# beecave-homelab/VibeVoice-ROCm

Measured on AMD Instinct MI355X. Metric: audio-sec/s, higher is better.
Workload: dtype bf16; 1 GPU; cfg2: VibeVoice-1.5B shapes, 1 speaker(s) x 203-frame voice prompt, 330-token prompt, 225 frames (30.0 s audio), CFG=2.0, 20 DPM-Solver++ steps, whole generate() incl. voice encode + prefill; global_batch=1, parallelism=replicas x1 (one dialogue per GPU), hipgraph=True

## Files before the change

### include/vv_hip.h

```cpp
#ifndef VV_HIP_H
#define VV_HIP_H

#include <stddef.h>
#include <stdint.h>

#ifdef __cplusplus
extern "C" {
#endif

typedef void* vv_stream_t;

enum { VV_F32 = 0, VV_BF16 = 1, VV_FP8 = 2  };
enum { VV_NF4 = 3 };
enum { VV_WQ_NF4 = 0x100 };
enum { VV_MXFP4 = 4 };
enum { VV_WQ_MXFP4 = 0x200 };
enum { VV_MXFP4_FRAG = 5 };
enum { VV_WQ_FRAG4 = 0x400 };
enum { VV_MXFP6 = 6 };
enum { VV_WQ_MXFP6 = 0x800 };
enum { VV_MXFP6_FRAG = 8 };
enum { VV_WQ_FRAG6 = 0x1000 };
enum { VV_OK = 0, VV_E_ARG = -1, VV_E_HIP = -2, VV_E_UNSUPPORTED = -3 };
enum { VV_PRO_NONE = 0, VV_PRO_RMSNORM = 1, VV_PRO_SILU = 2 };
// ... 122 lines not shown
                       const vv_sampler* sampler, const float* q, vv_stream_t stream);
int vv_llm_tail_batch_sample(const vv_llm* m, const float* h, int64_t ldh, int B, float* out, int64_t ldo, const void* w_valid, int nv, const int* ids,
                             float* logits_out, int* token_out, const int* forced_token, int* lens, int tok_start, int tok_diffusion,
                             int* frame_counter, const int* active, const vv_sampler* sampler, const float* q, vv_stream_t stream);
int vv_sample_ids(const float* logits, int n, const int* ids, const vv_sampler* sampler, const float* q, int* token_out, const int* forced_token,
                  vv_stream_t stream);

int vv_token_draws(float* q, int64_t ldq, int B, int nv, const uint64_t* seeds, const int* pos, int64_t ld_pos, int pos_bias, vv_stream_t stream);
int vv_llm_tail_sample_rows(const vv_llm* m, const float* h, int64_t ldh, int R, float* out, int64_t ldo, const void* w_valid, int nv, const int* ids,
                            float* logits_out, int* token_out, const int* forced_token, int* lens, int tok_start, int tok_diffusion, int* frame_counter,
                            const vv_sampler* samplers, const uint64_t* seeds, vv_stream_t stream);
int vv_llm_tail_batch_sample_rows(const vv_llm* m, const float* h, int64_t ldh, int B, float* out, int64_t ldo, const void* w_valid, int nv, const int* ids,
                                  float* logits_out, int* token_out, const int* forced_token, int* lens, int tok_start, int tok_diffusion,
                                  int* frame_counter, const int* active, const vv_sampler* samplers, const uint64_t* seeds, vv_stream_t stream);

typedef struct vv_head_layer {
  const float* norm_w;
  const void* wgate;
  const void* wup;
  const void* wdown;
  const void* adaln;
  vv_w8 q_gate, q_up, q_down;
  const void* f_gate; const void* f_up; const void* f_down;
} vv_head_layer;

typedef struct vv_head {
  int wdt, D, ffn, layers, latent, cond_dim;
  float eps;
  int flags;
  const void* noisy_proj;
  const void* cond_proj;
  const void* final_adaln;
  const void* final_linear;
  const vv_head_layer* layer;
  const float* fused_g;
} vv_head;

typedef struct vv_dpm_coef { float alpha_s, sigma_s, cx, cd, rinv; int order; float cn;  } vv_dpm_coef;

int vv_add_rows_silu(const float* a, int64_t lda, const float* b, int64_t ldb, float* out, int rows, int rows_b, int n, vv_stream_t stream);
int vv_add_rows_silu_bf16(const float* a, int64_t lda, const float* b, int64_t ldb, void* out, int rows, int rows_b, int n, vv_stream_t stream);
int vv_dpm_proj(const float* v, int64_t ldv, float cfg_scale, const vv_dpm_coef* coef, const float* x_in, const float* m_in,
                float* x_out, float* m_out, const void* w, int wdt, int latent, int D, float* h, int64_t ldh, int rows,
                const float* step_noise , vv_stream_t stream);

size_t vv_head_ws_bytes(const vv_head* h, int n_steps);
int vv_head_sample(const vv_head* h, const float* cond2, int64_t ld_cond, const float* noise, const float* temb,
                   const vv_dpm_coef* coef, int n_steps, float cfg_scale, float* latent_out, void* ws,
                   const float* sde_noise ,
                   vv_stream_t stream);
size_t vv_head_ws_bytes_batch(const vv_head* h, int n_steps, int B);
int vv_head_sample_batch(const vv_head* h, const float* cond, int64_t ld_cond, const float* noise, int64_t ld_noise, const float* temb,
                         const vv_dpm_coef* coef, int n_steps, float cfg_scale, float* latent_out, int64_t ld_latent, int B, void* ws,
                         vv_stream_t stream);
size_t vv_head_ws_bytes_batch_sde(const vv_head* h, int n_steps, int B);
int vv_head_sample_batch_sde(const vv_head* h, const float* cond, int64_t ld_cond, const float* noise, int64_t ld_noise, const float* temb,
                             const vv_dpm_coef* coef, int n_steps, float cfg_scale, float* latent_out, int64_t ld_latent, int B, void* ws,
                             const float* sde_noise, int64_t ld_sde, vv_stream_t stream);
int vv_head_sample_batch_cfg(const vv_head* h, const float* cond, int64_t ld_cond, const float* noise, int64_t ld_noise, const float* temb,
                             const vv_dpm_coef* coef, int n_steps, const float* cfg_rows , float* latent_out, int64_t ld_latent,
                             int B, void* ws, const float* sde_noise , int64_t ld_sde, vv_stream_t stream);
int vv_head_sample_route(const vv_head* h, const float* cond, int64_t ld_cond, const float* temb, const vv_dpm_coef* coef, int n_steps, int B,
                         int sde, const float* cfg_rows, const void* ws, char* name, int cap);
int vv_head_ws_layout(const vv_head* h, int n_steps, int B, int sde, int64_t* off, int cap);
int vv_noise_normal(float* noise, int64_t ld_noise, float* sde_noise, int64_t ld_sde, int B, int n, int n_steps, const uint64_t* seeds,
                    const int* frames, vv_stream_t stream);
int vv_head_forward(const vv_head* h, const float* x, const float* temb_rows, const float* cond, int R, float* v,
                    void* ws, vv_stream_t stream);

typedef struct vv_block {
  const float* gamma; const float* ffn_gamma; const float* norm_w; const float* ffn_norm_w;
  const float* dw_w;
  const float* dw_b;
  const void* w1; const float* b1;
  const void* w2; const float* b2;
  float* hist;
  vv_w8 q_w1, q_w2;
  const float* dw_last;
  float* hs;
} vv_block;

int vv_block1d(const struct vv_block* b, int wdt, const float* x, float* out, int T, int C, float eps, vv_stream_t stream);
int vv_block1d_route(const struct vv_block* b, int wdt, const float* x, const float* out, int T, int C, char* name, int cap);

size_t vv_block_mid_ws_bytes(int T, int C);
int vv_block_mid(const struct vv_block* b, int wdt, const float* x, float* out, void* ws, int T, int C, float eps, vv_stream_t stream);
int vv_block_mid_route(const struct vv_block* b, int wdt, const float* x, const float* out, const void* ws, int T, int C, char* name, int cap);

typedef struct vv_conv {
  const void* w;
  const float* b;
  int cin, cout, kk, stride, transposed;
  float* state;
} vv_conv;

#define VV_MAX_STAGES 8
typedef struct vv_convnet {
  int wdt, n_stages;
  float eps;
  vv_conv sample[VV_MAX_STAGES];
  int n_blocks[VV_MAX_STAGES];
  const vv_block* blocks[VV_MAX_STAGES];
  vv_conv head;
} vv_convnet;

size_t vv_convnet_ws_bytes(const vv_convnet* net, int64_t t_in, int decoder);
int vv_decoder_forward(const vv_convnet* net, const float* latent, int T, float pre_scale, float pre_bias, float* wav,
                       void* ws, vv_stream_t stream);
int vv_encoder_forward(const vv_convnet* net, const float* wav, int64_t T, float* feat, void* ws, vv_stream_t stream);
int vv_convnet_reset(const vv_convnet* net, vv_stream_t stream);

typedef struct vv_connector { int wdt, din, hidden; const void* fc1; const float* b1; const float* norm_w; const void* fc2; const float* b2; } vv_connector;
int vv_connector_forward(const vv_connector* c, const float* x, int R, float* out, int accumulate, float* ws, vv_stream_t stream);
int vv_connector_pair(const vv_connector* ac, const vv_connector* sem, const float* latent, const float* semfeat, float* out, int64_t ldo,
                      int rows_out, float* ws, vv_stream_t stream);

size_t vv_conv_rows_ws_bytes(const vv_convnet* net, int B, int decoder);
int vv_decoder_front_rows(const vv_convnet* const* nets, int B, const int* active, const float* latent, int64_t ld_latent,
                          float pre_scale, float pre_bias, float* mid, int64_t ld_mid, void* ws, vv_stream_t stream);
int vv_decoder_forward_from(const vv_convnet* net, const float* mid, float* wav, void* ws, vv_stream_t stream);
int vv_encoder_forward_until(const vv_convnet* net, const float* wav, int64_t T, float* mid, void* ws, vv_stream_t stream);
int vv_encoder_back_rows(const vv_convnet* const* nets, int B, const int* active, const float* mid, int64_t ld_mid,
                         float* feat, int64_t ld_feat, void* ws, vv_stream_t stream);
int vv_connector_pair_rows(const vv_connector* ac, const vv_connector* sem, const float* latent, int64_t ld_latent,
                           const float* semfeat, int64_t ld_feat, const int* active, float* out, int64_t ld_out,
                           int rows_out, int B, float* ws, vv_stream_t stream);

int vv_graph_begin(vv_stream_t stream);
int vv_graph_end(vv_stream_t stream, void** graph_exec_out);
int vv_graph_launch(void* graph_exec, vv_stream_t stream);
int vv_graph_destroy(void* graph_exec);

typedef struct vv_prof_entry { int m, n, k, dual, wdt, count; double total_ms; } vv_prof_entry;
int vv_prof_begin(int max_records);
int vv_prof_end(vv_prof_entry* out, int max_out, int* n_out);

typedef struct vv_nf4_src {
  const uint8_t* packed;
  const void* absmax;
  const float* quant_map;
  const float* nested_absmax;
  const float* nested_map;
  float nested_offset;
  int nested_blocksize;
  int n, k, blocksize;
} vv_nf4_src;
int vv_nf4_import(const vv_nf4_src* src, void* w, int64_t ldw, int row0, int rows_total, void* cq, float* cs, vv_stream_t stream);

#define VV_CONV_HOT_GEMV 0
#define VV_CONV_HOT_ROW 1
typedef struct vv_conv_hot_shape { const char* name; int kind, m, n, k, bias, gate, res; } vv_conv_hot_shape;
int vv_conv_hot_shapes(vv_conv_hot_shape* out, int cap);

size_t vv_sizeof(const char* struct_name);

#ifdef __cplusplus
}
#endif
#endif
```

### vibevoice_rocm_amd/_lib.py

```python
from __future__ import annotations

import ctypes as C
import os

_HERE = os.path.dirname(os.path.abspath(__file__))
LIB_PATH = os.path.join(_HERE, "libvv_hip.so")

VV_F32, VV_BF16, VV_FP8, VV_NF4, VV_MXFP4, VV_MXFP4_FRAG, VV_MXFP6 = 0, 1, 2, 3, 4, 5, 6
VV_MXFP6_FRAG = 8
VV_WQ_NF4 = 0x100
VV_WQ_MXFP4 = 0x200
VV_WQ_MXFP6 = 0x800
VV_WQ_FRAG4 = 0x400
VV_WQ_FRAG6 = 0x1000
PRO_NONE, PRO_RMSNORM, PRO_SILU = 0, 1, 2
ACT_NONE, ACT_GELU, ACT_SWIGLU = 0, 1, 2
LIN_X_BF16, LIN_OUT_BF16, LIN_W_REUSED, LIN_W_FRAG, LIN_PACKED, LIN_W_MXGEMM = 1, 2, 4, 8, 16, 32
LIN_W_MX6GEMM = 64
VV_MAX_STAGES = 8
KVQ_DERIVE_SCALES = 1

vp = C.c_void_p
i64 = C.c_int64

# ... 17 lines not shown

def kv_fp8_scale(absmax: float) -> float:
    import math
    a = abs(float(absmax))
    if a == 0.0:
        return 1.0
    m, e = math.frexp(a)
    return math.ldexp(1.0, e - 8 if m <= 0.875 else e - 7)


class LlmLayer(C.Structure):
    _fields_ = [("ln1", vp), ("ln2", vp), ("wqkv", vp), ("bqkv", vp), ("wo", vp), ("wgate", vp), ("wup", vp), ("wdown", vp),
                ("q_qkv", W8), ("q_o", W8), ("q_gate", W8), ("q_up", W8), ("q_down", W8),
                ("f_qkv", vp), ("f_o", vp), ("f_gate", vp), ("f_up", vp), ("f_down", vp)]


class Llm(C.Structure):
    _fields_ = [("wdt", C.c_int), ("hidden", C.c_int), ("inter", C.c_int), ("layers", C.c_int), ("heads", C.c_int),
                ("kv_heads", C.c_int), ("head_dim", C.c_int), ("rms_eps", C.c_float), ("inv_freq", vp),
                ("final_norm", vp), ("layer", C.POINTER(LlmLayer))]


class HeadLayer(C.Structure):
    _fields_ = [("norm_w", vp), ("wgate", vp), ("wup", vp), ("wdown", vp), ("adaln", vp), ("q_gate", W8), ("q_up", W8), ("q_down", W8),
                ("f_gate", vp), ("f_up", vp), ("f_down", vp)]


class Head(C.Structure):
    _fields_ = [("wdt", C.c_int), ("D", C.c_int), ("ffn", C.c_int), ("layers", C.c_int), ("latent", C.c_int),
                ("cond_dim", C.c_int), ("eps", C.c_float), ("flags", C.c_int), ("noisy_proj", vp), ("cond_proj", vp), ("final_adaln", vp),
                ("final_linear", vp), ("layer", C.POINTER(HeadLayer)), ("fused_g", vp)]


class DpmCoef(C.Structure):
    _fields_ = [("alpha_s", C.c_float), ("sigma_s", C.c_float), ("cx", C.c_float), ("cd", C.c_float),
                ("rinv", C.c_float), ("order", C.c_int), ("cn", C.c_float)]


class Block(C.Structure):
    _fields_ = [("gamma", vp), ("ffn_gamma", vp), ("norm_w", vp), ("ffn_norm_w", vp), ("dw_w", vp), ("dw_b", vp),
                ("w1", vp), ("b1", vp), ("w2", vp), ("b2", vp), ("hist", vp), ("q_w1", W8), ("q_w2", W8), ("dw_last", vp), ("hs", vp)]


class Conv(C.Structure):
    _fields_ = [("w", vp), ("b", vp), ("cin", C.c_int), ("cout", C.c_int), ("kk", C.c_int), ("stride", C.c_int),
                ("transposed", C.c_int), ("state", vp)]


class ConvNet(C.Structure):
    _fields_ = [("wdt", C.c_int), ("n_stages", C.c_int), ("eps", C.c_float), ("sample", Conv * VV_MAX_STAGES),
                ("n_blocks", C.c_int * VV_MAX_STAGES), ("blocks", C.POINTER(Block) * VV_MAX_STAGES), ("head", Conv)]


class Connector(C.Structure):
    _fields_ = [("wdt", C.c_int), ("din", C.c_int), ("hidden", C.c_int), ("fc1", vp), ("b1", vp), ("norm_w", vp),
                ("fc2", vp), ("b2", vp)]


class Nf4Src(C.Structure):
    _fields_ = [("packed", vp), ("absmax", vp), ("quant_map", vp), ("nested_absmax", vp), ("nested_map", vp), ("nested_offset", C.c_float),
                ("nested_blocksize", C.c_int), ("n", C.c_int), ("k", C.c_int), ("blocksize", C.c_int)]


class Sampler(C.Structure):
    _fields_ = [("temperature", C.c_float), ("top_k", C.c_int), ("top_p", C.c_float)]


class ProfEntry(C.Structure):
    _fields_ = [("m", C.c_int), ("n", C.c_int), ("k", C.c_int), ("dual", C.c_int), ("wdt", C.c_int), ("count", C.c_int),
                ("total_ms", C.c_double)]


_STRUCTS = dict(vv_w8=W8, vv_prof_entry=ProfEntry, vv_lin_args=LinArgs, vv_kv=KV, vv_llm_layer=LlmLayer, vv_llm=Llm, vv_head_layer=HeadLayer, vv_head=Head,
                vv_dpm_coef=DpmCoef, vv_block=Block, vv_conv=Conv, vv_convnet=ConvNet, vv_connector=Connector, vv_nf4_src=Nf4Src, vv_sampler=Sampler)

PROTOTYPES = {
    "vv_last_error": (C.c_char_p, []),
    "vv_abi_version": (C.c_int, []),
    "vv_init": (C.c_int, []),
    "vv_tune": (C.c_int, [C.c_char_p, C.c_int]),
    "vv_linear": (C.c_int, [C.POINTER(LinArgs), vp]),
    "vv_linear_route": (C.c_int, [C.POINTER(LinArgs), C.c_char_p, C.c_int]),
    "vv_rope_table": (C.c_int, [vp, vp, C.c_int, C.c_int, vp, vp]),
    "vv_rope_store": (C.c_int, [vp, i64, C.c_int, C.c_int, C.POINTER(KV), C.c_int, vp, vp, vp, vp]),
    "vv_attn": (C.c_int, [vp, i64, C.c_int, C.c_int, C.POINTER(KV), C.c_int, vp, vp, vp, i64, vp]),
    "vv_attn_route": (C.c_int, [vp, i64, C.c_int, C.c_int, C.POINTER(KV), vp, i64, C.c_char_p, C.c_int]),
    "vv_attn_decode": (C.c_int, [vp, i64, C.c_int, C.c_int, C.POINTER(KV), C.c_int, vp, vp, vp, i64, vp]),
    "vv_attn_decode_part_floats": (C.c_size_t, [C.c_int, C.c_int, C.c_int]),
    "vv_attn_decode_split": (C.c_int, [vp, i64, C.c_int, C.c_int, C.POINTER(KV), C.c_int, vp, vp, vp, i64, vp, vp, C.c_int, C.c_int, vp]),
    "vv_kv_quantize": (C.c_int, [C.POINTER(KV), C.POINTER(KV), C.c_int, C.c_int, C.c_int, C.c_int, vp]),
    "vv_kv_copy": (C.c_int, [C.POINTER(KV), C.c_int, C.POINTER(KV), C.c_int, C.c_int, vp]),
    "vv_block_mixer": (C.c_int, [vp, vp, C.c_int, C.c_int, vp, C.c_float, vp, vp, vp, vp, vp]),
    "vv_block_mixer_route": (C.c_int, [vp, vp, C.c_int, C.c_int, vp, vp, vp, vp, vp, C.c_char_p, C.c_int]),
    "vv_block1d": (C.c_int, [vp, C.c_int, vp, vp, C.c_int, C.c_int, C.c_float, vp]),
    "vv_block1d_route": (C.c_int, [vp, C.c_int, vp, vp, C.c_int, C.c_int, C.c_char_p, C.c_int]),
    "vv_block_mid_ws_bytes": (C.c_size_t, [C.c_int, C.c_int]),
    "vv_block_mid": (C.c_int, [vp, C.c_int, vp, vp, vp, C.c_int, C.c_int, C.c_float, vp]),
    "vv_block_mid_route": (C.c_int, [vp, C.c_int, vp, vp, vp, C.c_int, C.c_int, C.c_char_p, C.c_int]),
    "vv_conv_ctx": (C.c_int, [vp, vp, C.c_int, C.c_int, C.c_int, vp]),
    "vv_affine": (C.c_int, [vp, C.c_float, C.c_float, vp, i64, vp]),
    "vv_add_rows": (C.c_int, [vp, i64, vp, i64, vp, C.c_int, C.c_int, C.c_int, vp]),
    "vv_add_rows_silu": (C.c_int, [vp, i64, vp, i64, vp, C.c_int, C.c_int, C.c_int, vp]),
    "vv_add_rows_silu_bf16": (C.c_int, [vp, i64, vp, i64, vp, C.c_int, C.c_int, C.c_int, vp]),
    "vv_dpm_proj": (C.c_int, [vp, i64, C.c_float, C.POINTER(DpmCoef), vp, vp, vp, vp, vp, C.c_int, C.c_int, C.c_int, vp, i64, C.c_int, vp, vp]),
    "vv_embed_row": (C.c_int, [vp, C.c_int, i64, vp, vp, vp]),
    "vv_gather_rows": (C.c_int, [vp, C.c_int, i64, C.POINTER(C.c_int), C.c_int, vp, vp]),
    "vv_argmax_ids": (C.c_int, [vp, C.c_int, vp, vp, vp, vp]),
    "vv_cast_rows_bf16": (C.c_int, [vp, i64, C.c_int, C.c_int, C.c_int, vp, C.c_float, vp, i64, vp]),
    "vv_copy_rows": (C.c_int, [vp, i64, vp, i64, C.c_int, C.c_int, vp]),
    "vv_dpm_step": (C.c_int, [vp, i64, C.c_int, C.c_int, C.c_float, C.c_float, C.c_float, C.c_float, C.c_float,
                              C.c_float, C.c_int, vp, vp, vp]),
    "vv_advance_lens": (C.c_int, [vp, vp, C.c_int, C.c_int, vp, vp]),
    "vv_llm_ws_bytes": (C.c_size_t, [C.POINTER(Llm), C.c_int]),
    "vv_llm_forward": (C.c_int, [C.POINTER(Llm), C.POINTER(KV), vp, i64, C.c_int, vp, vp, vp, i64, vp, vp]),
    "vv_llm_prefill_packed_ws_bytes": (C.c_size_t, [C.POINTER(Llm), C.c_int]),
    "vv_llm_prefill_packed": (C.c_int, [C.POINTER(Llm), C.POINTER(KV), vp, i64, C.c_int, vp, vp, vp, C.c_int, vp, i64, vp, vp]),
    "vv_llm_tail": (C.c_int, [C.POINTER(Llm), vp, i64, C.c_int, vp, i64, vp, C.c_int, vp, vp, vp, vp, vp, C.c_int, C.c_int, vp, vp]),
    "vv_llm_tail_batch": (C.c_int, [C.POINTER(Llm), vp, i64, C.c_int, vp, i64, vp, C.c_int, vp, vp, vp, vp, vp, C.c_int, C.c_int, vp, vp, vp]),
    "vv_llm_tail_sample": (C.c_int, [C.POINTER(Llm), vp, i64, C.c_int, vp, i64, vp, C.c_int, vp, vp, vp, vp, vp, C.c_int, C.c_int, vp, C.POINTER(Sampler), vp, vp]),
    "vv_llm_tail_batch_sample": (C.c_int, [C.POINTER(Llm), vp, i64, C.c_int, vp, i64, vp, C.c_int, vp, vp, vp, vp, vp, C.c_int, C.c_int, vp, vp, C.POINTER(Sampler), vp, vp]),
    "vv_sample_ids": (C.c_int, [vp, C.c_int, vp, C.POINTER(Sampler), vp, vp, vp, vp]),
    "vv_token_draws": (C.c_int, [vp, i64, C.c_int, C.c_int, vp, vp, i64, C.c_int, vp]),
    "vv_llm_tail_sample_rows": (C.c_int, [C.POINTER(Llm), vp, i64, C.c_int, vp, i64, vp, C.c_int, vp, vp, vp, vp, vp, C.c_int, C.c_int, vp, vp, vp, vp]),
    "vv_llm_tail_batch_sample_rows": (C.c_int, [C.POINTER(Llm), vp, i64, C.c_int, vp, i64, vp, C.c_int, vp, vp, vp, vp, vp, C.c_int, C.c_int, vp, vp, vp, vp, vp]),
    "vv_head_ws_bytes": (C.c_size_t, [C.POINTER(Head), C.c_int]),
    "vv_head_ws_bytes_batch": (C.c_size_t, [C.POINTER(Head), C.c_int, C.c_int]),
    "vv_head_sample_batch": (C.c_int, [C.POINTER(Head), vp, i64, vp, i64, vp, C.POINTER(DpmCoef), C.c_int, C.c_float, vp, i64, C.c_int, vp, vp]),
    "vv_head_ws_bytes_batch_sde": (C.c_size_t, [C.POINTER(Head), C.c_int, C.c_int]),
    "vv_head_sample_batch_sde": (C.c_int, [C.POINTER(Head), vp, i64, vp, i64, vp, C.POINTER(DpmCoef), C.c_int, C.c_float, vp, i64, C.c_int, vp, vp, i64, vp]),
    "vv_head_sample_batch_cfg": (C.c_int, [C.POINTER(Head), vp, i64, vp, i64, vp, C.POINTER(DpmCoef), C.c_int, vp, vp, i64, C.c_int, vp, vp, i64, vp]),
    "vv_noise_normal": (C.c_int, [vp, i64, vp, i64, C.c_int, C.c_int, C.c_int, vp, vp, vp]),
    "vv_head_sample": (C.c_int, [C.POINTER(Head), vp, i64, vp, vp, C.POINTER(DpmCoef), C.c_int, C.c_float, vp, vp, vp, vp]),
    "vv_head_forward": (C.c_int, [C.POINTER(Head), vp, vp, vp, C.c_int, vp, vp, vp]),
    "vv_head_sample_route": (C.c_int, [C.POINTER(Head), vp, i64, vp, C.POINTER(DpmCoef), C.c_int, C.c_int, C.c_int, vp, vp, C.c_char_p, C.c_int]),
    "vv_head_ws_layout": (C.c_int, [C.POINTER(Head), C.c_int, C.c_int, C.c_int, C.POINTER(i64), C.c_int]),
    "vv_convnet_ws_bytes": (C.c_size_t, [C.POINTER(ConvNet), i64, C.c_int]),
    "vv_decoder_forward": (C.c_int, [C.POINTER(ConvNet), vp, C.c_int, C.c_float, C.c_float, vp, vp, vp]),
    "vv_encoder_forward": (C.c_int, [C.POINTER(ConvNet), vp, i64, vp, vp, vp]),
    "vv_convnet_reset": (C.c_int, [C.POINTER(ConvNet), vp]),
    "vv_connector_forward": (C.c_int, [C.POINTER(Connector), vp, C.c_int, vp, C.c_int, vp, vp]),
    "vv_connector_pair": (C.c_int, [C.POINTER(Connector), C.POINTER(Connector), vp, vp, vp, i64, C.c_int, vp, vp]),
    "vv_conv_rows_ws_bytes": (C.c_size_t, [C.POINTER(ConvNet), C.c_int, C.c_int]),
    "vv_decoder_front_rows": (C.c_int, [C.POINTER(C.POINTER(ConvNet)), C.c_int, vp, vp, i64, C.c_float, C.c_float, vp, i64, vp, vp]),
    "vv_decoder_forward_from": (C.c_int, [C.POINTER(ConvNet), vp, vp, vp, vp]),
    "vv_encoder_forward_until": (C.c_int, [C.POINTER(ConvNet), vp, i64, vp, vp, vp]),
    "vv_encoder_back_rows": (C.c_int, [C.POINTER(C.POINTER(ConvNet)), C.c_int, vp, vp, i64, vp, i64, vp, vp]),
    "vv_connector_pair_rows": (C.c_int, [C.POINTER(Connector), C.POINTER(Connector), vp, i64, vp, i64, vp, vp, i64, C.c_int, C.c_int, vp, vp]),
    "vv_graph_begin": (C.c_int, [vp]),
    "vv_graph_end": (C.c_int, [vp, C.POINTER(vp)]),
    "vv_graph_launch": (C.c_int, [vp, vp]),
    "vv_graph_destroy": (C.c_int, [vp]),
    "vv_nf4_import": (C.c_int, [C.POINTER(Nf4Src), vp, i64, C.c_int, C.c_int, vp, vp, vp]),
    "vv_conv_hot_shapes": (C.c_int, [vp, C.c_int]),
    "vv_sizeof": (C.c_size_t, [C.c_char_p]),
    "vv_prof_begin": (C.c_int, [C.c_int]),
    "vv_prof_end": (C.c_int, [C.POINTER(ProfEntry), C.c_int, C.POINTER(C.c_int)]),
}


class VVError(RuntimeError):
    pass


_lib = None


def load():
    global _lib
    if _lib is not None:
        return _lib
    import torch
    if not os.path.exists(LIB_PATH):
        raise VVError(f"{LIB_PATH} is missing: build the HIP extension first (python -m vibevoice_rocm_amd.build). "
                      "The MI355X kernels are the only compute path of this package.")
    lib = C.CDLL(LIB_PATH)
    for name, (res, args) in PROTOTYPES.items():
        fn = getattr(lib, name)
        fn.restype = res
        fn.argtypes = args
    for cname, cls in _STRUCTS.items():
        n = lib.vv_sizeof(cname.encode())
        if n != C.sizeof(cls):
            raise VVError(f"ABI mismatch for {cname}: C side {n} bytes, ctypes mirror {C.sizeof(cls)} bytes")
    _lib = lib
    return lib


def check(rc: int, what: str = ""):
    if rc != 0:
        raise VVError(f"{what} failed ({rc}): {load().vv_last_error().decode()}")


def ptr(t) -> int:
    return 0 if t is None else t.data_ptr()
```

### vibevoice_rocm_amd/build.py

```python
from __future__ import annotations

import hashlib
import os
import shutil
import subprocess
import sys

HERE = os.path.dirname(os.path.abspath(__file__))
ROOT = os.path.dirname(HERE)
SRC = [os.path.join(HERE, "csrc", f) for f in ("vv_kernels.hip", "vv_gemv_stream.hip", "vv_gemv_mx6.hip", "vv_gemv_hot.hip", "vv_conv_hot.hip", "vv_gemv_rows.hip", "vv_gemv_rows_mx6.hip", "vv_mfma_gemm.hip", "vv_gemm_packed.hip", "vv_gemm_mx.hip", "vv_gemm_mx6.hip", "vv_block1d.hip", "vv_convffn.hip",
                                               "vv_fused.hip", "vv_attn_decode.hip", "vv_attn_prefill.hip", "vv_model.hip",
                                               "vv_nf4_import.hip", "vv_kv_copy.hip", "vv_noise.hip")]
HDR = [os.path.join(ROOT, "include", "vv_hip.h"), os.path.join(HERE, "csrc", "vv_common.h"), os.path.join(HERE, "csrc", "vv_device.h"),
       os.path.join(HERE, "csrc", "vv_head_boundary.inc"),
       os.path.join(HERE, "csrc", "vv_gemv_rows.h"), os.path.join(HERE, "csrc", "vv_gemv_rows_body.inc"), os.path.join(HERE, "csrc", "vv_gemv_rows_tile.inc"),
       os.path.join(HERE, "csrc", "vv_llm_tail.inc"), os.path.join(HERE, "csrc", "vv_llm_tail_fast.inc")]
OUT = os.path.join(HERE, "libvv_hip.so")
OBJDIR = os.path.join(HERE, "csrc", "build")
STAMP = os.path.join(HERE, "libvv_hip.stamp")
FLAGS = ["--offload-arch=gfx950", "-O3", "-std=c++17", "-fPIC"]
PRELOAD = ["-mllvm", "-amdgpu-kernarg-preload-count=16"]
UNIT_FLAGS = {"vv_gemv_hot.hip": PRELOAD}


def find_hipcc() -> str:
    for c in (os.environ.get("HIPCC"), shutil.which("hipcc"), "/opt/rocm/bin/hipcc"):
        if c and os.path.exists(c):
            return c
    raise RuntimeError("hipcc not found (ROCm toolchain required to build the MI355X kernels)")


def _flavour() -> str:
    return hashlib.sha256("\n".join([os.path.basename(s) for s in SRC] + FLAGS + [u + " " + " ".join(f) for u, f in sorted(UNIT_FLAGS.items())]).encode()).hexdigest()[:16]


def _check_sources():
    missing = [p for p in SRC + HDR if not os.path.exists(p)]
    if missing:
        raise RuntimeError("missing kernel sources: " + ", ".join(os.path.relpath(p, ROOT) for p in missing))


def up_to_date() -> bool:
    if not os.path.exists(OUT):
        return False
    if not all(os.path.exists(p) for p in SRC + HDR):
        return True
    t = os.path.getmtime(OUT)
    if not all(os.path.getmtime(p) <= t for p in SRC + HDR):
        return False
    try:
        return open(STAMP).read().strip() == _flavour()
    except OSError:
        return False


def _obj(src: str) -> str:
    return os.path.join(OBJDIR, os.path.basename(src) + ".o")


def build(force: bool = False, verbose: bool = True, jobs: int = 6) -> str:
    if not force and up_to_date():
        return OUT
    _check_sources()
    os.makedirs(OBJDIR, exist_ok=True)
    flags = [*FLAGS, "-I" + os.path.join(ROOT, "include"), "-I" + os.path.join(HERE, "csrc")]
    hipcc = find_hipcc()
    hdr_t = max(os.path.getmtime(p) for p in HDR)
    todo = [s for s in SRC if force or not os.path.exists(_obj(s)) or os.path.getmtime(_obj(s)) < max(os.path.getmtime(s), hdr_t)]
    procs = []
    for s in todo:
        cmd = [hipcc, *flags, *UNIT_FLAGS.get(os.path.basename(s), []), "-c", s, "-o", _obj(s)]
        if verbose:
            print(" ".join(cmd), flush=True)
        procs.append((s, subprocess.Popen(cmd)))
        while sum(p.poll() is None for _, p in procs) >= jobs:
            next(p for _, p in procs if p.poll() is None).wait()
    failed = [s for s, p in procs if p.wait() != 0]
    if failed:
        raise RuntimeError("hipcc failed for " + ", ".join(os.path.basename(f) for f in failed))
    cmd = [hipcc, "--offload-arch=gfx950", "-shared", "-fPIC", *[_obj(s) for s in SRC], "-o", OUT]
    if verbose:
        print(" ".join(cmd), flush=True)
    subprocess.run(cmd, check=True)
    with open(STAMP, "w") as f:
        f.write(_flavour() + "\n")
    return OUT


if __name__ == "__main__":
    build(force="--force" in sys.argv)
    print(OUT)
```

### vibevoice_rocm_amd/csrc/vv_common.h

```cpp
#ifndef VV_COMMON_H
#define VV_COMMON_H
#include <hip/hip_runtime.h>
#include <stdarg.h>
#include <stdint.h>
#include "vv_hip.h"

int vv_set_error(int code, const char* fmt, ...);

#define VV_CHECK_LAUNCH(name)                                                                    \
  do {                                                                                           \
    hipError_t e_ = hipGetLastError();                                                           \
    if (e_ != hipSuccess) return vv_set_error(VV_E_HIP, "%s: %s", name, hipGetErrorString(e_));  \
  } while (0)

#define VV_TRY(expr)            \
  do {                          \
    int rc_ = (expr);           \
    if (rc_) return rc_;        \
  } while (0)

struct vv_kv_args {
  void* k; void* v;
  int kvdt, layers, rows, kv_heads, s_max, head_dim;
  void* vt;
  vv_kv_args(const vv_kv& a) : k(a.k), v(a.v), kvdt(a.kvdt), layers(a.layers), rows(a.rows), kv_heads(a.kv_heads), s_max(a.s_max), head_dim(a.head_dim), vt(a.vt) {}
};
struct vv_kv_args8 : vv_kv_args {
  const float* kscale; const float* vscale;
  vv_kv_args8(const vv_kv& a) : vv_kv_args(a), kscale(a.kscale), vscale(a.vscale) {}
};

static constexpr struct { int bit, wq, frag_bit, frag_wdt; } VV_WQ_KINDS[] = {
  {VV_WQ_MXFP6, VV_MXFP6, VV_WQ_FRAG6, VV_MXFP6_FRAG},
  {VV_WQ_MXFP4, VV_MXFP4, VV_WQ_FRAG4, VV_MXFP4_FRAG},
  {VV_WQ_NF4, VV_NF4, 0, 0},
};
constexpr int vv_wq_bits() { int bits = VV_WQ_FRAG4 | VV_WQ_FRAG6; for (const auto& k : VV_WQ_KINDS) bits |= k.bit; return bits; }
struct vv_wq_kind { int wq; int fragq; };
static inline vv_wq_kind vv_wq_strip(int* wdt) {
  vv_wq_kind r = {VV_FP8, 0};
  for (const auto& k : VV_WQ_KINDS) if (*wdt & k.bit) { r.wq = k.wq; break; }
  for (const auto& k : VV_WQ_KINDS) if (r.wq == k.wq && k.frag_bit && (*wdt & k.frag_bit)) r.fragq = k.frag_wdt;
  *wdt &= ~vv_wq_bits();
  return r;
}
const char* vv_gemv_stream_refusal(const vv_lin_args& a, int* rc);
const char* vv_gemv_mx6_refusal(const vv_lin_args& a, int* rc);
const char* vv_gemv_rows_refusal(const vv_lin_args& a, int* rc);
const char* vv_gemv_rows_mx6_refusal(const vv_lin_args& a, int* rc);

enum { VV_GEMV_STREAM = 1, VV_GEMV_HOT = 2, VV_GEMV_CONV_HOT = 3 };
struct vv_stream_route { int kind, idx, m, dual, ksplit, ku, rw, wq, n_groups, blocks, threads; };
vv_stream_route vv_gemv_stream_decide(const vv_lin_args& a);
int vv_launch_gemv_stream_route(const vv_lin_args& a, const vv_stream_route& r, hipStream_t s);
int vv_gemv_stream_route_name(const vv_stream_route& r, char* name, int cap);
struct vv_mx6_route { int kind, m, dual, ksplit, ku, n_groups, blocks, threads; };
vv_mx6_route vv_gemv_mx6_decide(const vv_lin_args& a);
int vv_launch_gemv_mx6_route(const vv_lin_args& a, const vv_mx6_route& r, hipStream_t s);
int vv_gemv_mx6_route_name(const vv_mx6_route& r, char* name, int cap);
void vv_gemv_mx6_set_blocks(int b);
struct vv_gemv_hot_shape { const char* name; int m, n, k, dual, pro, mod, bias, gate, res, act, flags; };
extern "C" int vv_gemv_hot_shapes(vv_gemv_hot_shape* out, int cap);
int vv_gemv_hot_covers(const vv_lin_args& a);
int vv_launch_gemv_hot(const vv_lin_args& a, int idx, hipStream_t s);
void vv_gemv_hot_set(int mask);
int vv_conv_hot_gemv_covers(const vv_lin_args& a);
int vv_launch_conv_hot_gemv(const vv_lin_args& a, int idx, hipStream_t s);
int vv_launch_conv_hot_row(const vv_block& B, const float* x, float* y, float* hidden, float* hist_new, int C, float eps, hipStream_t s);
void vv_conv_hot_set(int mask);
int vv_launch_gemv_rows(const vv_lin_args& a, float* part, size_t part_floats, int* tickets, size_t n_tickets, hipStream_t s);
struct vv_rows_route { int kind, dual, nw, ks, pers, wf, ksplit, spw, atomic, n_groups, gx, rt; };
vv_rows_route vv_gemv_rows_decide(const vv_lin_args& a, bool have_ws, size_t part_floats, size_t n_tickets);
int vv_launch_gemv_rows_route(const vv_lin_args& a, const vv_rows_route& r, float* part, int* tickets, hipStream_t s);
int vv_gemv_rows_route_name(const vv_rows_route& r, char* name, int cap);
size_t vv_gemv_rows_part_floats(int n, int dual);
size_t vv_gemv_rows_tickets(int n);
int vv_gemv_rows_init();
bool vv_gemv_rows_mx6_built(int dual, int nw, int ks, int pers);
int vv_launch_gemv_rows_mx6_route(const vv_lin_args& a, const vv_rows_route& r, float* part, int* tickets, hipStream_t s);
int vv_gemv_rows_mx6_init();
void vv_gemv_rows_set(int on, int blocks, int pers);
int vv_linear_ws(const vv_lin_args* a, const void* f1, const void* f2, float* part, size_t part_floats, int* tickets, size_t n_tickets,
                 vv_stream_t stream, const vv_w8* q1 = nullptr, const vv_w8* q2 = nullptr, int fragq = 0);
int vv_launch_mfma_gemm(const vv_lin_args& a, hipStream_t s);
enum { VV_MFMA_STREAM = 1, VV_MFMA_TILED = 2 };
struct vv_mfma_route { int kind, dual, ksplit, xb, mt, bk, tm; };
vv_mfma_route vv_mfma_decide(const vv_lin_args& a);
int vv_launch_mfma_route(const vv_lin_args& a, const vv_mfma_route& r, hipStream_t s);
int vv_mfma_route_name(const vv_mfma_route& r, char* name, int cap);
int vv_mfma_gemm_init();
bool vv_gemm_packed_covers(const vv_lin_args& a);
int vv_launch_gemm_packed(const vv_lin_args& a, hipStream_t s);
int vv_gemm_packed_route_name(const vv_lin_args& a, char* name, int cap);
void vv_gemm_packed_set_rows(int rows);
int vv_gemm_packed_init();
int vv_gemm_mx_check(const vv_lin_args& a);
int vv_launch_gemm_mx(const vv_lin_args& a, hipStream_t s);
int vv_gemm_mx_route_name(const vv_lin_args& a, char* name, int cap);
int vv_gemm_mx6_check(const vv_lin_args& a);
int vv_launch_gemm_mx6(const vv_lin_args& a, hipStream_t s);
int vv_gemm_mx6_route_name(const vv_lin_args& a, char* name, int cap);
int vv_launch_attn_decode(const float* qkv, int64_t ld_qkv, int R, int heads, const vv_kv* kv, int layer, const float2* rope, const int* lens, float* out,
                          int64_t ldo, float* part, int* tickets, int nsplit, int part_cap, hipStream_t s);
int vv_attn_decode_ws(const float* qkv, int64_t ld_qkv, int R, int heads, const vv_kv* kv, int layer, const float* rope_table, const int* lens, float* out,
                      int64_t ldo, float* part, int* tickets, int nsplit, int part_cap, vv_stream_t stream);
int vv_launch_kv_quantize(const vv_kv* src, const vv_kv* dst, int src_row, int dst_row, int len, int flags, hipStream_t s);
bool vv_attn_prefill_covers(const float* qkv, int64_t ld_qkv, int R, const vv_kv* kv, const float* out, int64_t ldo);
int vv_launch_attn_prefill(const float* qkv, int64_t ld_qkv, int R, int heads, const vv_kv* kv, int layer, const int* lens, const int* cache_rows,
                           float* out, int64_t ldo, hipStream_t s);
int vv_head_init_fused(const vv_head* h, const float* noise, float* Xs, float* Ms, float* h0, int64_t ldh, hipStream_t s);
bool vv_head_boundary_supported(const vv_head* h);
int vv_head_boundary_fused(const vv_head* h, const float* hrows, int64_t ldh, const float* shift, const float* scale, int64_t ld_mod, float cfg,
                           const vv_dpm_coef* k, float* Xs, float* Ms, float* h_out, int64_t ldh_out, float* latent_out, hipStream_t s);
int vv_head_boundary_batch(const vv_head* h, const float* hrows, int64_t ldh, const float* shift, const float* scale, int64_t ld_mod, float cfg,
                           const vv_dpm_coef* k, float* Xs, float* Ms, int64_t state_stride, float* h_out, int64_t ldh_out, float* latent_out,
                           int64_t latent_stride, int B, hipStream_t s,
                           const float* nx = nullptr, int64_t nx_stride = 0,
                           const float* cfg_rows = nullptr);
int vv_head_sde_proj_fused(const vv_head* h, const float* sde_noise, int64_t ld_sde, int n_steps, int B, float* NX, hipStream_t s);
int vv_fused_init();
int vv_head_pre_fused(const vv_head* h, const float* cond2, int64_t ld_cond, const float* temb, int n_steps, void* c_bf16, const float* noise,
                      float* Xs, float* Ms, float* h0, int64_t ldh, hipStream_t s);
int vv_launch_connector_pair(const vv_connector* ac, const vv_connector* sem, const float* latent, const float* semfeat, float* out, int64_t ldo, int rows_out,
                             float* ws, hipStream_t s);
int vv_head_modulations_fused(const vv_head* h, const void* c_bf16, int rows, float* const* mod, float* modf, hipStream_t s);
int vv_head_pre_decide(const vv_head* h, const float* cond2, int64_t ld_cond, const float* temb, int n_steps, const void* c_bf16);
int vv_head_modulations_decide(const vv_head* h, const void* c_bf16, int rows);
int vv_head_boundary_decide(const vv_head* h);
struct vv_conv_ctx_item { float* pad; float* state; int ctx, T, C; const float* dw_w; float* hs; int affine; float scale, bias; };
int vv_conv_ctx_batch(const vv_conv_ctx_item* items, int n, int scatter, hipStream_t s);
struct vv_rows_delta { int64_t d[8]; };
enum { VV_ROWS_W2 = 0, VV_ROWS_DEC = 1, VV_ROWS_SEM = 2 };
int vv_launch_row_in_rows(const vv_block& B, int nb, const float* x, float* y, float* hidden, float* hist_new, const vv_rows_delta& dl, const int* active,
                          float eps, hipStream_t s);
int vv_launch_rows_gemv(int shape, int nb, const float* x, int64_t ldx, const void* w, const float* bias, const float* gate, const float* res,
                        int64_t ldres, float* out, int64_t ldo, const int* active, hipStream_t s);
struct vv_rows_item { float* buf; int64_t ld_buf; float* other; int64_t ld_other; int relocate, n, C; const float* dw_w; float* hs; int affine; float scale, bias; };
#define VV_ROWS_ITEMS 24
int vv_launch_rows_ctx(const vv_rows_item* items, int n, int nb, const vv_rows_delta& dl, const int* active, int scatter, hipStream_t s);
int vv_launch_rows_bcast(const float* src, int64_t ld_src, float* out, int64_t ldo, int rows_out, int n, int nb, const int* active, hipStream_t s);
int vv_block1d_init();
int vv_launch_block1d(const vv_block& B, int wdt, const float* x, float* out, int T, int C, float eps, hipStream_t s);
void vv_block1d_set_fused(int on);
void vv_block1d_set_blocks(int b);
int vv_convffn_init();
int vv_launch_convffn(const vv_block& B, int wdt, const float* x, float* y, void* hidden, float* hist_new, float* out, int T, int C, float eps,
                      hipStream_t s);
void vv_convffn_set(int on);
int vv_launch_ffn_in_row(const vv_block& B, int wdt, const float* x, float* y, float* hidden, float* hist_new, int C, float eps, hipStream_t s);
void vv_convffn_set_t1(int on);
int vv_launch_ffn_in_row_hs(const vv_block& B, int wdt, const float* x, float* y, float* hidden, float* hist_new, int C, float eps, hipStream_t s);
void vv_convffn_set_t1hs(int on);
void vv_convffn_set_rows(int c, int rows);
void vv_convffn_set_c128(int on);
bool vv_convffn_prefers(int wdt, int T, int C);
int vv_launch_skinny(const vv_lin_args& a, hipStream_t s);
struct vv_skinny_route { int kind, nst, nb; };
vv_skinny_route vv_skinny_decide(const vv_lin_args& a);
int vv_skinny_route_name(const vv_skinny_route& r, char* name, int cap);
bool vv_skinny_covers(const vv_lin_args& a);
void vv_skinny_set(int on, int min_m, int max_m);
int vv_rmsnorm_rows(const float* x, int64_t ldx, const float* w, float eps, int rows, int n, float* out, int64_t ldo, hipStream_t s,
                    const int* sel = nullptr);

#ifdef __HIPCC__
__host__ __device__ __forceinline__ unsigned vv_e4m3_sat(float x) {
  union { float f; unsigned u; } a, t;
  a.f = x;
  const unsigned sign = (a.u >> 24) & 0x80u;
  a.u &= 0x7fffffffu;
  if (!(a.f < 448.f)) a.f = 448.f;
  if (a.u < 0x3c800000u) {
    t.f = a.f * 512.f + 8388608.f;
    return sign | (t.u & 0xffu);
  }
  const unsigned r = (a.u + 0x7ffffu + ((a.u >> 20) & 1u)) >> 20;
  return sign | (r - ((127u - 7u) << 3));
}
__device__ __forceinline__ float vv_gelu_as(float v) {
  const float x = v * 0.70710678118654752440f, ax = fabsf(x);
  const float t = __builtin_amdgcn_rcpf(fmaf(0.3275911f, ax, 1.0f));
  const float poly = t * fmaf(t, fmaf(t, fmaf(t, fmaf(t, 1.061405429f, -1.453152027f), 1.421413741f), -0.284496736f), 0.254829592f);
  const float erf_abs = 1.0f - poly * __expf(-ax * ax);
  return 0.5f * v * (1.0f + copysignf(erf_abs, x));
}

struct philox4 { unsigned x, y, z, w; };

__host__ __device__ __forceinline__ unsigned mulhi32(unsigned a, unsigned b) { return (unsigned)(((unsigned long long)a * b) >> 32); }

__host__ __device__ __forceinline__ philox4 philox4x32_10(philox4 c, unsigned k0, unsigned k1) {
  constexpr unsigned M0 = 0xD2511F53u, M1 = 0xCD9E8D57u, W0 = 0x9E3779B9u, W1 = 0xBB67AE85u;
#pragma unroll
  for (int r = 0; r < 10; ++r) {
    const unsigned hi0 = mulhi32(M0, c.x), lo0 = M0 * c.x, hi1 = mulhi32(M1, c.z), lo1 = M1 * c.z;
    c = philox4{hi1 ^ c.y ^ k0, lo1, hi0 ^ c.w ^ k1, lo0};
    k0 += W0;
    k1 += W1;
  }
  return c;
}

__device__ __forceinline__ float noise_uniform(unsigned x) { return (float)x * 0x1p-32f + 0x1p-33f; }

__device__ __forceinline__ float vv_token_draw_exp(unsigned x) {
  const float q = -logf(noise_uniform(x));
  return q > 0.f ? q : 0x1p-126f;
}
__device__ __forceinline__ float4 vv_token_draw(uint64_t seed, unsigned p, unsigned j) {
  const philox4 x = philox4x32_10(philox4{j, p, 0u, 1u}, (unsigned)(seed & 0xffffffffu), (unsigned)(seed >> 32));
  return make_float4(vv_token_draw_exp(x.x), vv_token_draw_exp(x.y), vv_token_draw_exp(x.z), vv_token_draw_exp(x.w));
}
__device__ __forceinline__ void vv_token_draws8(uint64_t seed, unsigned p, int nv, float (&q)[8]) {
  const float4 a = vv_token_draw(seed, p, 0u);
  float4 b = make_float4(1.f, 1.f, 1.f, 1.f);
  if (nv > 4) b = vv_token_draw(seed, p, 1u);
  const float v[8] = {a.x, a.y, a.z, a.w, b.x, b.y, b.z, b.w};
#pragma unroll
  for (int i = 0; i < 8; ++i) q[i] = i < nv ? v[i] : 1.f;
}

__device__ __forceinline__ int vv_sample_choice(const float (&l)[8], int nv, const vv_sampler sp, const float (&q)[8]) {
// ... 78 lines not shown
```

### vibevoice_rocm_amd/csrc/vv_conv_hot.hip

```cpp
#include <hip/hip_runtime.h>
#include <hip/hip_bf16.h>
#include <stdint.h>

#include "vv_hip.h"
#include "vv_common.h"
#include "vv_device.h"

namespace {

template <int N, int K, int NW, int R, bool GR>
__global__ __launch_bounds__(64 * NW) void conv_gemv_kernel(const vv_lin_args a) {
  constexpr int KU = K / (512 * NW);
  static_assert(K % (512 * NW) == 0 && N % R == 0 && R <= 64 && R * KU + 2 * KU + 3 < 63, "whole units, whole row sets, every load in flight at once");
  __shared__ float part[NW][R];
  const int tid = threadIdx.x, lane = tid & 63;
  const int wave = __builtin_amdgcn_readfirstlane(tid >> 6);
  const int n0 = (int)blockIdx.x * R;
  const bf16_t* __restrict__ W = reinterpret_cast<const bf16_t*>(a.w);

  int koff[KU];
#pragma unroll
  for (int u = 0; u < KU; ++u) koff[u] = (wave + NW * u) * 512 + lane * 8;
  float4 xa[KU], xb[KU];
#pragma unroll
// ... 154 lines not shown
    if (lane == 0) part[wave] = q;
    __syncthreads();
    const float rstd1 = rsqrtf(((part[0] + part[1]) + (part[2] + part[3])) / (float)C + eps);
#pragma unroll
    for (int j = 0; j < 2; ++j) {
      float xn[4];
#pragma unroll
      for (int e = 0; e < 4; ++e) xn[e] = xv[j][e] * rstd1 * nw[j][e];
#pragma unroll
      for (int r = 0; r < 5; ++r) st4(hn + (size_t)r * C + c0[j], hrow[r][j]);
      st4(hn + (size_t)5 * C + c0[j], xn);
    }
    return;
  }

  const int n0 = blockIdx.x * 32;
  const int lm = lane & 31, hk = (lane >> 5) * 8;
  float xv[BT][2][4], hsv[BT][2][4];
  float dwl[2][4], nw[2][4], db[2][4], gm[2][4], fw[2][4];
#pragma unroll
  for (int j = 0; j < 2; ++j) {
#pragma unroll
    for (int b = 0; b < BT; ++b) ld4(x + (size_t)b * C + c0[j], xv[b][j]);
    ld4(B.norm_w + c0[j], nw[j]);
#pragma unroll
    for (int b = 0; b < BT; ++b) {
      const float* hs = B.hs;
      if constexpr (BT > 1) hs += dl.d[b];
      ld4(hs + c0[j], hsv[b][j]);
    }
    ld4(B.dw_last + c0[j], dwl[j]);
    ld4(B.dw_b + c0[j], db[j]);
    ld4(B.gamma + c0[j], gm[j]);
    ld4(B.ffn_norm_w + c0[j], fw[j]);
  }
  u32x4 wf[ST];
  {
    const bf16_t* wr = reinterpret_cast<const bf16_t*>(B.w1) + (int64_t)(n0 + lm) * C + wave * (C / 4) + hk;
#pragma unroll
    for (int s = 0; s < ST; ++s) wf[s] = ldw<NT>(wr + s * 16);
  }
  const float b1v = B.b1[n0 + lm];
  __builtin_amdgcn_sched_barrier(0);
#pragma unroll
  for (int b = 0; b < BT; ++b) {
    float q = 0.f;
#pragma unroll
    for (int j = 0; j < 2; ++j)
#pragma unroll
      for (int e = 0; e < 4; ++e) q = fmaf(xv[b][j][e], xv[b][j][e], q);
    q = vv_wave_sum(q);
    if (lane == 0) part[b * 8 + wave] = q;
  }
  __syncthreads();
#pragma unroll
  for (int b = 0; b < BT; ++b) {
    const float* pb = part + b * 8;
    const float rstd1 = rsqrtf(((pb[0] + pb[1]) + (pb[2] + pb[3])) / (float)C + eps);
    float q2 = 0.f;
#pragma unroll
    for (int j = 0; j < 2; ++j)
#pragma unroll
      for (int e = 0; e < 4; ++e) {
        const float xn = xv[b][j][e] * rstd1 * nw[j][e];
        const float sc = db[j][e] + hsv[b][j][e] + dwl[j][e] * xn;
        xv[b][j][e] = xv[b][j][e] + gm[j][e] * sc;
        q2 = fmaf(xv[b][j][e], xv[b][j][e], q2);
      }
    q2 = vv_wave_sum(q2);
    if (lane == 0) part[b * 8 + 4 + wave] = q2;
  }
  __syncthreads();
  {
    const int ys0 = blockIdx.x * (C / ROW_WG);
#pragma unroll
    for (int b = 0; b < BT; ++b) {
      const float* pb = part + b * 8 + 4;
      const float rstd2 = rsqrtf(((pb[0] + pb[1]) + (pb[2] + pb[3])) / (float)C + eps);
#pragma unroll
      for (int j = 0; j < 2; ++j) {
        uint2 p;
        p.x = pack2(xv[b][j][0] * rstd2 * fw[j][0], xv[b][j][1] * rstd2 * fw[j][1]);
        p.y = pack2(xv[b][j][2] * rstd2 * fw[j][2], xv[b][j][3] * rstd2 * fw[j][3]);
        *reinterpret_cast<uint2*>(xh + b * P1 + c0[j]) = p;
        if (c0[j] >= ys0 && c0[j] < ys0 + C / ROW_WG) st4(y + (size_t)b * C + c0[j], xv[b][j]);
      }
    }
  }
  __syncthreads();
  f32x16 acc;
#pragma unroll
  for (int i = 0; i < 16; ++i) acc[i] = 0.f;
  {
    const bf16_t* xf = xh + min(lm, BT - 1) * P1 + wave * (C / 4) + hk;
#pragma unroll
    for (int s = 0; s < ST; ++s) {
      const u32x4 xb = *reinterpret_cast<const u32x4*>(xf + s * 16);
      acc = __builtin_amdgcn_mfma_f32_32x32x16_bf16(__builtin_bit_cast(bf16x8, wf[s]), __builtin_bit_cast(bf16x8, xb), acc, 0, 0, 0);
    }
  }
  if (lm < BT) {
#pragma unroll
    for (int r = 0; r < 16; ++r) red[((wave * 16 + r) * 2 + (lane >> 5)) * BT + lm] = acc[r];
  }
  __syncthreads();
  if (tid < 32 * BT) {
    const int b = tid >> 5, o = tid & 31;
    const int r = 4 * (o >> 3) + (o & 3), h = (o >> 2) & 1;
    float s = 0.f;
#pragma unroll
    for (int w4 = 0; w4 < 4; ++w4) s += red[((w4 * 16 + r) * 2 + h) * BT + b];
    hidden[(size_t)b * 4 * C + n0 + o] = vv_gelu_as(s + b1v);
  }
}

struct CtxRowsArgs { vv_rows_item it[VV_ROWS_ITEMS]; vv_rows_delta dl; int n; };

__global__ __launch_bounds__(256) void rows_ctx_kernel(const CtxRowsArgs a, const int* __restrict__ active, int scatter) {
  const vv_rows_item it = a.it[blockIdx.y];
  const int b = blockIdx.z;
  if (scatter && !active[b]) return;
  float* buf = it.buf + (int64_t)b * it.ld_buf;
  float* oth = it.other + (it.relocate ? a.dl.d[b] : (int64_t)b * it.ld_other);
  const int n = it.n;
  if (!scatter) {
    if (it.affine) {
      for (int i = blockIdx.x * 256 + threadIdx.x; i < n; i += gridDim.x * 256) buf[i] = fmaf(oth[i], it.scale, it.bias);
      return;
    }
    for (int i = blockIdx.x * 256 + threadIdx.x; i < n; i += gridDim.x * 256) buf[i] = oth[i];
    return;
  }
  for (int i = blockIdx.x * 256 + threadIdx.x; i < n; i += gridDim.x * 256) oth[i] = buf[i];
  if (it.hs) {
    float* hs = it.hs + a.dl.d[b];
    for (int c = blockIdx.x * 256 + threadIdx.x; c < it.C; c += gridDim.x * 256) {
      float s = 0.f;
#pragma unroll
      for (int k = 0; k < 6; ++k) s = fmaf(it.dw_w[(size_t)c * 7 + k], buf[(size_t)k * it.C + c], s);
      hs[c] = s;
    }
  }
}

__global__ __launch_bounds__(256) void rows_bcast_kernel(const float* __restrict__ src, int64_t ld_src, float* __restrict__ out, int64_t ldo, int rows_out, int n,
                                                         const int* __restrict__ active) {
  const int b = blockIdx.y;
  if (active && !active[b]) return;
  for (int i = blockIdx.x * 256 + threadIdx.x; i < n; i += gridDim.x * 256) {
    const float v = src[(int64_t)b * ld_src + i];
    for (int r = 0; r < rows_out; ++r) out[((int64_t)b * rows_out + r) * ldo + i] = v;
  }
}

constexpr int N_HOT = 4;
const vv_conv_hot_shape g_table[N_HOT] = {
    {"block.w2",         VV_CONV_HOT_GEMV, 1, 2048, 8192,  1,   1,   1},
    {"block.ffn_in_row", VV_CONV_HOT_ROW,  1, 8192, 2048,  1,   0,   0},
    {"dec.handover",     VV_CONV_HOT_GEMV, 1, 8192, 4096,  1,   0,   0},
    {"sem.handover",     VV_CONV_HOT_GEMV, 1, 2048, 16384, 1,   0,   0},
};

constexpr int HOT_DEFAULT = 0xf;
int g_hot = HOT_DEFAULT;

bool matches(const vv_conv_hot_shape& e, const vv_lin_args& a) {
  return e.kind == VV_CONV_HOT_GEMV && a.m == e.m && a.n == e.n && a.k == e.k && a.wdt == VV_BF16 && !a.w2 && a.pro == VV_PRO_NONE && !a.mod_scale &&
         !a.mod_shift && (a.bias != nullptr) == (e.bias != 0) && (a.gate != nullptr) == (e.gate != 0) && (!e.gate || a.gate_ld == 0) &&
         (a.res != nullptr) == (e.res != 0) && a.act == VV_ACT_NONE && a.flags == 0;
}

bool a16(const void* q) { return q && ((uintptr_t)q % 16) == 0; }

}

void vv_conv_hot_set(int mask) { g_hot = mask < 0 ? HOT_DEFAULT : mask; }

extern "C" int vv_conv_hot_shapes(vv_conv_hot_shape* out, int cap) {
  for (int i = 0; i < N_HOT && i < cap; ++i) out[i] = g_table[i];
  return N_HOT;
}

int vv_conv_hot_gemv_covers(const vv_lin_args& a) {
  if (!(g_hot & ((1 << N_HOT) - 1)) || a.m != 1 || a.wdt != VV_BF16) return -1;
  for (int i = 0; i < N_HOT; ++i)
    if ((g_hot >> i & 1) && matches(g_table[i], a)) return i;
  return -1;
}

int vv_launch_conv_hot_gemv(const vv_lin_args& a, int id, hipStream_t s) {
  const bool alt = (g_hot & 256) != 0;
  switch (id) {
    case 0:
      if (alt) hipLaunchKernelGGL((conv_gemv_kernel<2048, 8192, 4, 4, true>), dim3(512), dim3(256), 0, s, a);
      else hipLaunchKernelGGL((conv_gemv_kernel<2048, 8192, 4, 8, true>), dim3(256), dim3(256), 0, s, a);
      return 1;
    case 2:
      if (alt) hipLaunchKernelGGL((conv_gemv_kernel<8192, 4096, 4, 16, false>), dim3(512), dim3(256), 0, s, a);
      else hipLaunchKernelGGL((conv_gemv_kernel<8192, 4096, 4, 8, false>), dim3(1024), dim3(256), 0, s, a);
      return 1;
    case 3:
      if (alt) hipLaunchKernelGGL((conv_gemv_kernel<2048, 16384, 8, 8, false>), dim3(256), dim3(512), 0, s, a);
      else hipLaunchKernelGGL((conv_gemv_kernel<2048, 16384, 8, 4, false>), dim3(512), dim3(512), 0, s, a);
      return 1;
  }
  return 0;
}

int vv_launch_conv_hot_row(const vv_block& B, const float* x, float* y, float* hidden, float* hist_new, int C, float eps, hipStream_t s) {
  if (!(g_hot & 2) || C != ROW_C || !hist_new) return 0;
  const vv_rows_delta none{};
  const int* active = nullptr;
  if (!(g_hot & 512)) hipLaunchKernelGGL((row_in_rows_kernel<1, false>), dim3(ROW_WG + 1), dim3(256), 0, s, x, y, hidden, hist_new, B, eps, none, active);
  else hipLaunchKernelGGL((row_in_rows_kernel<1, true>), dim3(ROW_WG + 1), dim3(256), 0, s, x, y, hidden, hist_new, B, eps, none, active);
  return 1;
}

int vv_launch_row_in_rows(const vv_block& B, int nb, const float* x, float* y, float* hidden, float* hist_new, const vv_rows_delta& dl, const int* active,
                          float eps, hipStream_t s) {
  if (!a16(B.w1) || !a16(B.b1) || !a16(B.gamma) || !a16(B.norm_w) || !a16(B.ffn_norm_w) || !a16(B.dw_b) || !a16(B.dw_last) || !a16(B.hs) || !a16(B.hist) ||
      !a16(x) || !a16(y) || !a16(hidden) || !a16(hist_new) || !active || x == y)
    return vv_set_error(VV_E_ARG, "vv_conv_rows: misaligned or missing operand of the one-row block");
  for (int b = 0; b < nb; ++b)
    if (dl.d[b] % 4) return vv_set_error(VV_E_ARG, "vv_conv_rows: dialogue %d's state is not 16-byte aligned to dialogue 0's", b);
#define VV_RIR(BT) case BT: hipLaunchKernelGGL((row_in_rows_kernel<BT, false>), dim3(ROW_WG + BT), dim3(256), 0, s, x, y, hidden, hist_new, B, eps, dl, active); break
  switch (nb) {
    VV_RIR(2); VV_RIR(3); VV_RIR(4); VV_RIR(5); VV_RIR(6); VV_RIR(7); VV_RIR(8);
    default: return vv_set_error(VV_E_UNSUPPORTED, "vv_conv_rows: %d rows (2..8)", nb);
  }
#undef VV_RIR
  VV_CHECK_LAUNCH("row_in_rows");
  return 0;
}

int vv_launch_rows_gemv(int shape, int nb, const float* x, int64_t ldx, const void* w, const float* bias, const float* gate, const float* res,
                        int64_t ldres, float* out, int64_t ldo, const int* active, hipStream_t s) {
  if (!a16(x) || !a16(w) || !bias || !out || ldx % 4 || (shape == VV_ROWS_W2 && (!gate || !res)))
    return vv_set_error(VV_E_ARG, "vv_conv_rows: misaligned or missing operand of a %d-row GEMV", nb);
  const bf16_t* W = reinterpret_cast<const bf16_t*>(w);
#define VV_RG(BT, N, K, NW, R, GR, HB) \
  hipLaunchKernelGGL((rows_gemv_kernel<BT, N, K, NW, R, GR, HB>), dim3(N / R), dim3(64 * NW), 0, s, x, ldx, W, bias, gate, res, ldres, out, ldo, active)
#define VV_RGS(BT)                                                      \
  case BT:                                                              \
    if (shape == VV_ROWS_W2) VV_RG(BT, 2048, 8192, 4, 4, true, BT);     \
    else if (shape == VV_ROWS_DEC) VV_RG(BT, 8192, 4096, 4, 8, false, BT); \
    else VV_RG(BT, 2048, 16384, 8, 4, false, (BT >= 7 ? 2 : BT == 6 ? 3 : BT)); \
    break
  if (shape != VV_ROWS_W2 && shape != VV_ROWS_DEC && shape != VV_ROWS_SEM) return vv_set_error(VV_E_ARG, "vv_conv_rows: GEMV shape %d", shape);
  switch (nb) {
    VV_RGS(2); VV_RGS(3); VV_RGS(4); VV_RGS(5); VV_RGS(6); VV_RGS(7); VV_RGS(8);
    default: return vv_set_error(VV_E_UNSUPPORTED, "vv_conv_rows: %d rows (2..8)", nb);
  }
#undef VV_RGS
#undef VV_RG
  VV_CHECK_LAUNCH("rows_gemv");
  return 0;
}

int vv_launch_rows_ctx(const vv_rows_item* items, int n, int nb, const vv_rows_delta& dl, const int* active, int scatter, hipStream_t s) {
  if (n <= 0) return 0;
  if (n > VV_ROWS_ITEMS || nb < 1 || nb > 8 || (scatter && !active)) return vv_set_error(VV_E_ARG, "vv_conv_rows: state move list");
  CtxRowsArgs a;
  a.n = n; a.dl = dl;
  int mx = 0;
  for (int i = 0; i < n; ++i) { a.it[i] = items[i]; if (items[i].n > mx) mx = items[i].n; }
  for (int i = n; i < VV_ROWS_ITEMS; ++i) a.it[i] = vv_rows_item{};
  int bx = (mx + 1023) / 1024;
  if (bx > 16) bx = 16;
  if (bx < 1) bx = 1;
  hipLaunchKernelGGL(rows_ctx_kernel, dim3(bx, n, nb), dim3(256), 0, s, a, active, scatter);
  VV_CHECK_LAUNCH("rows_ctx");
  return 0;
}

int vv_launch_rows_bcast(const float* src, int64_t ld_src, float* out, int64_t ldo, int rows_out, int n, int nb, const int* active, hipStream_t s) {
  hipLaunchKernelGGL(rows_bcast_kernel, dim3((n + 255) / 256 < 16 ? (n + 255) / 256 : 16, nb), dim3(256), 0, s, src, ld_src, out, ldo, rows_out, n, active);
  VV_CHECK_LAUNCH("rows_bcast");
  return 0;
}
```

### vibevoice_rocm_amd/csrc/vv_convffn.hip

```cpp
#include <hip/hip_runtime.h>
#include <hip/hip_bf16.h>
#include <stdint.h>

#include "vv_hip.h"
#include "vv_common.h"
#include "vv_device.h"

namespace {


#ifdef VV_CF_TIMING
__device__ unsigned long long g_cf_t[8];
#define CSTAMP(i) do { if (blockIdx.x == 0 && blockIdx.y == 0 && threadIdx.x == 0) { const long long t_ = wall_clock64(); g_cf_t[i] += (unsigned long long)(t_ - tprev_); tprev_ = t_; } } while (0)
#else
#define CSTAMP(i) do { } while (0)
#endif

constexpr int TR2 = 16;
constexpr int HALO = 6;

__device__ __forceinline__ float sq4(const float4 v) { return v.x * v.x + v.y * v.y + v.z * v.z + v.w * v.w; }

template <int C, int TRV, int NT = 256> struct InLay {
  static constexpr int VW = C >= 256 ? 4 : 2;
  static constexpr int F4 = C / 4;
  static constexpr int FV = C / VW;
  static constexpr int TPR = FV < NT ? FV : NT;
  static constexpr int NWV = NT / 64;
  static constexpr int CPT = FV / TPR;
  static constexpr int RP = NT / TPR;
  static constexpr int NI = (TRV + HALO + RP - 1) / RP;
  static constexpr int WR = NI * RP;
  static constexpr int WPR = TPR / 64;
  static constexpr int P1 = C + 8;
  static constexpr int ST = C / (16 * NWV);
  static constexpr size_t XN = (size_t)WR * C * 4;
  static constexpr size_t RED = (size_t)NWV * 16 * 64 * 4;
  static constexpr size_t XH = (size_t)(WR - HALO) * P1 * 2;
  static constexpr size_t PART = (size_t)2 * WR * 8 * 4;
  static constexpr size_t LDS = (XN > RED ? XN : RED) + XH + PART;
};

template <int VW> __device__ __forceinline__ void ldv(const float* p, float (&o)[VW]) {
  if constexpr (VW == 4) { const float4 t = *reinterpret_cast<const float4*>(p); o[0] = t.x; o[1] = t.y; o[2] = t.z; o[3] = t.w; }
  else { const float2 t = *reinterpret_cast<const float2*>(p); o[0] = t.x; o[1] = t.y; }
}
template <int VW> __device__ __forceinline__ void stv(float* p, const float (&o)[VW]) {
  if constexpr (VW == 4) *reinterpret_cast<float4*>(p) = make_float4(o[0], o[1], o[2], o[3]);
  else *reinterpret_cast<float2*>(p) = make_float2(o[0], o[1]);
}

template <int C, int TRV, bool HF32, int NT>
__global__ __launch_bounds__(NT) void ffn_in_kernel(const float* __restrict__ x, float* __restrict__ y, void* __restrict__ hidden_v,
                                                     float* __restrict__ hist_new, int T, const vv_block B, float eps) {
  using L = InLay<C, TRV, NT>;
  constexpr int TR = TRV, CPT = L::CPT, VW = L::VW, NWV = L::NWV;
#ifdef VV_CF_TIMING
  long long tprev_ = wall_clock64();
#endif
  extern __shared__ __attribute__((aligned(16))) unsigned char smem[];
  float* xn = reinterpret_cast<float*>(smem);
  float* red = reinterpret_cast<float*>(smem);
  bf16_t* xh = reinterpret_cast<bf16_t*>(smem + (L::XN > L::RED ? L::XN : L::RED));
  float* part = reinterpret_cast<float*>(smem + (L::XN > L::RED ? L::XN : L::RED) + L::XH);
  float* part2 = part + L::WR * 8;
  const int tid = threadIdx.x, lane = tid & 63, wave = __builtin_amdgcn_readfirstlane(tid >> 6);
  const int n0 = blockIdx.x * 32;
  const int t0 = blockIdx.y * TR;
  const int rows = min(TR, T - t0);
  const int lm = lane & 31, hk = (lane >> 5) * 8;

  const int rloc = wave / L::WPR, slot = wave % L::WPR;
  int c0[CPT];
#pragma unroll
  for (int j = 0; j < CPT; ++j) c0[j] = VW * (tid % L::TPR + L::TPR * j);
  const float* hb = B.hist ? B.hist : x;
  const float hkeep = B.hist ? 1.f : 0.f;
  float own[L::NI][CPT][VW];
#pragma unroll
  for (int i = 0; i < L::NI; ++i) {
    const int w = rloc + L::RP * i, t = t0 - HALO + w;
    const bool isx = t >= 0;
    const float* src = isx ? x + (int64_t)min(t, T - 1) * C : hb + (int64_t)(B.hist ? HALO + t : 0) * C;
    const float keep = (w < rows + HALO) ? (isx ? 1.f : hkeep) : 0.f;
#pragma unroll
    for (int j = 0; j < CPT; ++j) {
      ldv<VW>(src + c0[j], own[i][j]);
#pragma unroll
      for (int e = 0; e < VW; ++e) own[i][j][e] *= keep;
    }
  }
  float nw[CPT][VW], db[CPT][VW], gm[CPT][VW], fw[CPT][VW];
  float tap[CPT][VW * 7];
#pragma unroll
  for (int j = 0; j < CPT; ++j) {
    ldv<VW>(B.norm_w + c0[j], nw[j]);
    ldv<VW>(B.dw_b + c0[j], db[j]);
    ldv<VW>(B.gamma + c0[j], gm[j]);
    ldv<VW>(B.ffn_norm_w + c0[j], fw[j]);
#pragma unroll
    for (int q = 0; q < 7; ++q) {
      float tq[VW];
      ldv<VW>(B.dw_w + (size_t)c0[j] * 7 + VW * q, tq);
#pragma unroll
      for (int e = 0; e < VW; ++e) tap[j][VW * q + e] = tq[e];
    }
  }
  u32x4 wf[L::ST];
  {
    const bf16_t* wr = reinterpret_cast<const bf16_t*>(B.w1) + (int64_t)(n0 + lm) * C + wave * (C / NWV) + hk;
#pragma unroll
    for (int s = 0; s < L::ST; ++s) wf[s] = *reinterpret_cast<const u32x4*>(wr + s * 16);
  }
  const int eg = wave & 3;
  const float4 b1v = *reinterpret_cast<const float4*>(B.b1 + n0 + 8 * eg + 4 * (lane >> 5));
  __builtin_amdgcn_sched_barrier(0);

  CSTAMP(0);
#pragma unroll
  for (int i = 0; i < L::NI; ++i) {
    const int w = rloc + L::RP * i;
    float q = 0.f;
#pragma unroll
    for (int j = 0; j < CPT; ++j)
#pragma unroll
      for (int e = 0; e < VW; ++e) q = fmaf(own[i][j][e], own[i][j][e], q);
    const float s = vv_wave_sum(q);
    if (lane == 0) part[w * 8 + slot] = s;
  }
  __syncthreads();
  CSTAMP(1);
#pragma unroll
  for (int i = 0; i < L::NI; ++i) {
    const int w = rloc + L::RP * i, t = t0 - HALO + w;
    float ss = part[w * 8];
#pragma unroll
    for (int sl = 1; sl < L::WPR; ++sl) ss += part[w * 8 + sl];
    const bool isx = t >= 0;
    const float rstd = isx ? rsqrtf(ss / (float)C + eps) : 1.f;
#pragma unroll
    for (int j = 0; j < CPT; ++j) {
      float o[VW];
#pragma unroll
      for (int e = 0; e < VW; ++e) o[e] = own[i][j][e] * rstd * (isx ? nw[j][e] : 1.f);
      stv<VW>(xn + w * C + c0[j], o);
    }
  }
  __syncthreads();
  CSTAMP(2);

  float y1[L::NI][CPT][VW];
#pragma unroll
  for (int i = 0; i < L::NI; ++i) {
#pragma unroll
    for (int j = 0; j < CPT; ++j)
#pragma unroll
      for (int e = 0; e < VW; ++e) y1[i][j][e] = 0.f;
    if (L::RP * i + L::RP - 1 < HALO) continue;
    const int w = rloc + L::RP * i, tt = w - HALO;
    const int tc = max(tt, 0);
    const float ok = (tt >= 0 && tt < rows) ? 1.f : 0.f;
    float q = 0.f;
#pragma unroll
    for (int j = 0; j < CPT; ++j) {
      float s[VW];
#pragma unroll
      for (int e = 0; e < VW; ++e) s[e] = db[j][e];
#pragma unroll
      for (int k = 0; k < 7; ++k) {
        float v[VW];
        ldv<VW>(xn + (tc + k) * C + c0[j], v);
#pragma unroll
        for (int e = 0; e < VW; ++e) s[e] = fmaf(tap[j][7 * e + k], v[e], s[e]);
      }
#pragma unroll
      for (int e = 0; e < VW; ++e) {
        y1[i][j][e] = (own[i][j][e] + gm[j][e] * s[e]) * ok;
        q = fmaf(y1[i][j][e], y1[i][j][e], q);
      }
    }
    const float s2 = vv_wave_sum(q);
    if (lane == 0) part2[w * 8 + slot] = s2;
  }
  if (hist_new && blockIdx.x == 0 && t0 + TR >= T) {
    for (int e = tid; e < HALO * L::F4; e += NT) {
      const int j = e / L::F4, c4 = e - j * L::F4;
      *reinterpret_cast<float4*>(hist_new + (size_t)j * C + 4 * c4) = *reinterpret_cast<const float4*>(xn + (size_t)(T - t0 + j) * C + 4 * c4);
    }
  }
  __syncthreads();
  CSTAMP(3);
  {
    const int ys0 = blockIdx.x * (C / (int)gridDim.x);
#pragma unroll
    for (int i = 0; i < L::NI; ++i) {
      if (L::RP * i + L::RP - 1 < HALO) continue;
      const int w = rloc + L::RP * i, tt = w - HALO;
      if (tt >= 0) {
        float ss = part2[w * 8];
#pragma unroll
        for (int sl = 1; sl < L::WPR; ++sl) ss += part2[w * 8 + sl];
        const float rstd = rsqrtf(ss / (float)C + eps);
#pragma unroll
        for (int j = 0; j < CPT; ++j) {
          if constexpr (VW == 4) {
            uint2 p;
            p.x = pack2(y1[i][j][0] * rstd * fw[j][0], y1[i][j][1] * rstd * fw[j][1]);
            p.y = pack2(y1[i][j][2] * rstd * fw[j][2], y1[i][j][3] * rstd * fw[j][3]);
            *reinterpret_cast<uint2*>(xh + tt * L::P1 + c0[j]) = p;
          } else {
            *reinterpret_cast<unsigned int*>(xh + tt * L::P1 + c0[j]) = pack2(y1[i][j][0] * rstd * fw[j][0], y1[i][j][1] * rstd * fw[j][1]);
          }
          const bool mine = c0[j] >= ys0 && c0[j] < ys0 + C / (int)gridDim.x;
          if (mine && tt < rows) stv<VW>(y + (int64_t)(t0 + tt) * C + c0[j], y1[i][j]);
        }
      }
    }
  }
  __syncthreads();

  CSTAMP(4);
  f32x16 acc;
#pragma unroll
  for (int i = 0; i < 16; ++i) acc[i] = 0.f;
  {
    const bf16_t* xf = xh + min(lm, TR - 1) * L::P1 + wave * (C / NWV) + hk;
#pragma unroll
    for (int s = 0; s < L::ST; ++s) {
      const u32x4 xb = *reinterpret_cast<const u32x4*>(xf + s * 16);
      acc = __builtin_amdgcn_mfma_f32_32x32x16_bf16(__builtin_bit_cast(bf16x8, wf[s]), __builtin_bit_cast(bf16x8, xb), acc, 0, 0, 0);
    }
  }
#pragma unroll
  for (int r = 0; r < 16; ++r) red[(wave * 16 + r) * 64 + lane] = acc[r];
  __syncthreads();
  CSTAMP(5);
  {
    const int m = lane & 31;
    if (m < rows && wave < 4) {
      float v[4];
#pragma unroll
      for (int i = 0; i < 4; ++i) {
        float s = 0.f;
#pragma unroll
        for (int w4 = 0; w4 < NWV; ++w4) s += red[(w4 * 16 + 4 * eg + i) * 64 + lane];
        v[i] = s;
      }
      const float g0 = vv_gelu_as(v[0] + b1v.x), g1 = vv_gelu_as(v[1] + b1v.y), g2 = vv_gelu_as(v[2] + b1v.z), g3 = vv_gelu_as(v[3] + b1v.w);
      const int64_t ho = (int64_t)(t0 + m) * (4 * C) + n0 + 8 * eg + 4 * (lane >> 5);
      if (HF32) {
        *reinterpret_cast<float4*>(reinterpret_cast<float*>(hidden_v) + ho) = make_float4(g0, g1, g2, g3);
      } else {
        uint2 p;
        p.x = pack2(g0, g1);
        p.y = pack2(g2, g3);
        *reinterpret_cast<uint2*>(reinterpret_cast<bf16_t*>(hidden_v) + ho) = p;
      }
    }
  }
  CSTAMP(6);
}


__global__ __launch_bounds__(256) void ffn_in_row_kernel(const float* __restrict__ x, float* __restrict__ y, float* __restrict__ hidden,
                                                         float* __restrict__ hist_new, const vv_block B, float eps) {
  constexpr int C = 2048, P1 = C + 8, ST = C / 64;
  __shared__ __attribute__((aligned(16))) bf16_t xh[P1];
  __shared__ float red[4 * 16 * 64];
  __shared__ float part[8];
  const int tid = threadIdx.x, lane = tid & 63, wave = __builtin_amdgcn_readfirstlane(tid >> 6);
  const int n0 = blockIdx.x * 32;
  const int lm = lane & 31, hk = (lane >> 5) * 8;
  float xv[2][4], hsv[2][4], dl[2][4], nw[2][4], db[2][4], gm[2][4], fw[2][4];
  int c0[2];
#pragma unroll
  for (int j = 0; j < 2; ++j) {
    c0[j] = 4 * (tid + 256 * j);
    ldv<4>(x + c0[j], xv[j]);
    ldv<4>(B.norm_w + c0[j], nw[j]);
    ldv<4>(B.hs + c0[j], hsv[j]);
    ldv<4>(B.dw_last + c0[j], dl[j]);
    ldv<4>(B.dw_b + c0[j], db[j]);
    ldv<4>(B.gamma + c0[j], gm[j]);
    ldv<4>(B.ffn_norm_w + c0[j], fw[j]);
  }
  const bool keeper = hist_new && blockIdx.x == 0;
  float hrow[5][2][4];
  if (keeper) {
#pragma unroll
    for (int r = 0; r < 5; ++r)
#pragma unroll
      for (int j = 0; j < 2; ++j) ldv<4>(B.hist + (size_t)(r + 1) * C + c0[j], hrow[r][j]);
  }
  u32x4 wf[ST];
  {
    const bf16_t* wr = reinterpret_cast<const bf16_t*>(B.w1) + (int64_t)(n0 + lm) * C + wave * (C / 4) + hk;
#pragma unroll
    for (int s = 0; s < ST; ++s) wf[s] = *reinterpret_cast<const u32x4*>(wr + s * 16);
  }
  const int eg = wave;
  const float4 b1v = *reinterpret_cast<const float4*>(B.b1 + n0 + 8 * eg + 4 * (lane >> 5));
  __builtin_amdgcn_sched_barrier(0);
  float q = 0.f;
#pragma unroll
  for (int j = 0; j < 2; ++j)
#pragma unroll
    for (int e = 0; e < 4; ++e) q = fmaf(xv[j][e], xv[j][e], q);
  q = vv_wave_sum(q);
  if (lane == 0) part[wave] = q;
  __syncthreads();
  const float rstd1 = rsqrtf(((part[0] + part[1]) + (part[2] + part[3])) / (float)C + eps);
  float yv[2][4], xn[2][4];
  float q2 = 0.f;
#pragma unroll
  for (int j = 0; j < 2; ++j)
#pragma unroll
    for (int e = 0; e < 4; ++e) {
      xn[j][e] = xv[j][e] * rstd1 * nw[j][e];
      const float sc = db[j][e] + hsv[j][e] + dl[j][e] * xn[j][e];
      yv[j][e] = xv[j][e] + gm[j][e] * sc;
      q2 = fmaf(yv[j][e], yv[j][e], q2);
    }
  q2 = vv_wave_sum(q2);
  if (lane == 0) part[4 + wave] = q2;
  if (keeper) {
#pragma unroll
    for (int j = 0; j < 2; ++j) {
#pragma unroll
      for (int r = 0; r < 5; ++r) stv<4>(hist_new + (size_t)r * C + c0[j], hrow[r][j]);
      stv<4>(hist_new + (size_t)5 * C + c0[j], xn[j]);
    }
  }
  __syncthreads();
  const float rstd2 = rsqrtf(((part[4] + part[5]) + (part[6] + part[7])) / (float)C + eps);
  {
    const int ys0 = blockIdx.x * (C / (int)gridDim.x);
#pragma unroll
    for (int j = 0; j < 2; ++j) {
      uint2 p;
      p.x = pack2(yv[j][0] * rstd2 * fw[j][0], yv[j][1] * rstd2 * fw[j][1]);
      p.y = pack2(yv[j][2] * rstd2 * fw[j][2], yv[j][3] * rstd2 * fw[j][3]);
      *reinterpret_cast<uint2*>(xh + c0[j]) = p;
      if (c0[j] >= ys0 && c0[j] < ys0 + C / (int)gridDim.x) stv<4>(y + c0[j], yv[j]);
    }
  }
  __syncthreads();
  f32x16 acc;
#pragma unroll
  for (int i = 0; i < 16; ++i) acc[i] = 0.f;
  {
    const bf16_t* xf = xh + wave * (C / 4) + hk;
#pragma unroll
    for (int s = 0; s < ST; ++s) {
      const u32x4 xb = *reinterpret_cast<const u32x4*>(xf + s * 16);
      acc = __builtin_amdgcn_mfma_f32_32x32x16_bf16(__builtin_bit_cast(bf16x8, wf[s]), __builtin_bit_cast(bf16x8, xb), acc, 0, 0, 0);
    }
  }
#pragma unroll
  for (int r = 0; r < 16; ++r) red[(wave * 16 + r) * 64 + lane] = acc[r];
  __syncthreads();
  if ((lane & 31) == 0) {
    float v[4];
#pragma unroll
    for (int i = 0; i < 4; ++i) {
      float s = 0.f;
#pragma unroll
      for (int w4 = 0; w4 < 4; ++w4) s += red[(w4 * 16 + 4 * eg + i) * 64 + lane];
      v[i] = s;
    }
    *reinterpret_cast<float4*>(hidden + n0 + 8 * eg + 4 * (lane >> 5)) =
        make_float4(vv_gelu_as(v[0] + b1v.x), vv_gelu_as(v[1] + b1v.y), vv_gelu_as(v[2] + b1v.z), vv_gelu_as(v[3] + b1v.w));
  }
}

template <int C, int NW>
__global__ __launch_bounds__(64 * NW) void ffn_out_kernel(const bf16_t* __restrict__ hidden, const float* res, float* out, const float* __restrict__ hist_new,
                                                          int T, const vv_block B) {
  constexpr int K = 4 * C, KW = K / NW, ST = KW / 32;
  __shared__ float red[NW * 4 * 64];
  const int tid = threadIdx.x, lane = tid & 63, wave = tid >> 6;
  const int n0 = blockIdx.x * 16, t0 = blockIdx.y * TR2;
  const int r16 = lane & 15, kq = lane >> 4;
  u32x4 wf[ST], hf[ST];
  {
    const bf16_t* wr = reinterpret_cast<const bf16_t*>(B.w2) + (int64_t)(n0 + r16) * K + wave * KW + 8 * kq;
    const bf16_t* hr = hidden + (int64_t)min(t0 + r16, T - 1) * K + wave * KW + 8 * kq;
#pragma unroll
    for (int s = 0; s < ST; ++s) {
      wf[s] = *reinterpret_cast<const u32x4*>(wr + s * 32);
      hf[s] = *reinterpret_cast<const u32x4*>(hr + s * 32);
    }
  }
  const int ei = (tid >> 6) & 3, el = tid & 63;
  const int en = n0 + 4 * (el >> 4) + ei, em = t0 + (el & 15);
  const bool ev = em < T && tid < 256;
  const float b2v = B.b2[en], fgv = B.ffn_gamma[en];
  const float rv = ev ? res[(int64_t)em * C + en] : 0.f;
  const bool mover = hist_new && B.hist && blockIdx.x == 0 && blockIdx.y == 0;
  constexpr int HN = (HALO * C / 4 + 64 * NW - 1) / (64 * NW);
  float4 hv[HN];
  if (mover) {
#pragma unroll
    for (int i = 0; i < HN; ++i) {
      const int e = tid + 64 * NW * i;
      hv[i] = e < HALO * C / 4 ? *reinterpret_cast<const float4*>(hist_new + 4 * (size_t)e) : make_float4(0.f, 0.f, 0.f, 0.f);
    }
  }
  f32x4 acc = {0.f, 0.f, 0.f, 0.f};
#pragma unroll
  for (int s = 0; s < ST; ++s)
    acc = __builtin_amdgcn_mfma_f32_16x16x32_bf16(__builtin_bit_cast(bf16x8, wf[s]), __builtin_bit_cast(bf16x8, hf[s]), acc, 0, 0, 0);
#pragma unroll
  for (int i = 0; i < 4; ++i) red[(wave * 4 + i) * 64 + lane] = acc[i];
  __syncthreads();
  if (ev) {
    float s = 0.f;
#pragma unroll
    for (int w4 = 0; w4 < NW; ++w4) s += red[(w4 * 4 + ei) * 64 + el];
    out[(int64_t)em * C + en] = rv + fgv * (s + b2v);
  }
  if (mover) {
#pragma unroll
    for (int i = 0; i < HN; ++i) {
      const int e = tid + 64 * NW * i;
      if (e < HALO * C / 4) *reinterpret_cast<float4*>(B.hist + 4 * (size_t)e) = hv[i];
    }
  }
}

template <int NST, int NB>
__global__ __launch_bounds__(256) void skinny_kernel(const float* __restrict__ x, int64_t ldx, int M, const bf16_t* __restrict__ W, int K,
                                                     const float* __restrict__ bias, float* __restrict__ out, int64_t ldo) {
  __shared__ float red[4 * 4 * 64];
  const int tid = threadIdx.x, lane = tid & 63, wave = tid >> 6;
  const int n0 = blockIdx.x * 16, t0 = blockIdx.y * 16;
  const int r16 = lane & 15, kq = lane >> 4;
  const int kb = wave * (32 * NST * NB) + 8 * kq;
  const bf16_t* wr = W + (int64_t)(n0 + r16) * K + kb;
  const float* xr = x + (int64_t)min(t0 + r16, M - 1) * ldx + kb;
  const int ei = tid >> 6, el = tid & 63;
  const int en = n0 + 4 * (el >> 4) + ei, em = t0 + (el & 15);
  const float bv = bias ? bias[en] : 0.f;
  f32x4 acc = {0.f, 0.f, 0.f, 0.f};
#pragma unroll
  for (int b = 0; b < NB; ++b) {
    u32x4 wf[NST];
    float4 xa[NST], xb[NST];
#pragma unroll
    for (int s = 0; s < NST; ++s) {
      wf[s] = *reinterpret_cast<const u32x4*>(wr + 32 * (b * NST + s));
      xa[s] = *reinterpret_cast<const float4*>(xr + 32 * (b * NST + s));
      xb[s] = *reinterpret_cast<const float4*>(xr + 32 * (b * NST + s) + 4);
    }
#pragma unroll
    for (int s = 0; s < NST; ++s) {
      u32x4 p;
      p.x = pack2(xa[s].x, xa[s].y); p.y = pack2(xa[s].z, xa[s].w); p.z = pack2(xb[s].x, xb[s].y); p.w = pack2(xb[s].z, xb[s].w);
      acc = __builtin_amdgcn_mfma_f32_16x16x32_bf16(__builtin_bit_cast(bf16x8, wf[s]), __builtin_bit_cast(bf16x8, p), acc, 0, 0, 0);
    }
  }
#pragma unroll
  for (int i = 0; i < 4; ++i) red[(wave * 4 + i) * 64 + lane] = acc[i];
  __syncthreads();
  if (em < M) {
    float v = 0.f;
#pragma unroll
    for (int w4 = 0; w4 < 4; ++w4) v += red[(w4 * 4 + ei) * 64 + el];
    out[(int64_t)em * ldo + en] = v + bv;
  }
}

int g_skinny = 1, g_skinny_min_m = 5, g_skinny_max_m = 2048;

int g_on = 1;

constexpr int in_threads_of(int c) { return (c == 512 || c == 1024) ? 512 : 256; }
template <int C> constexpr int in_threads() { return in_threads_of(C); }

template <int C, int TRV, int NW>
int launch_c(const vv_block& B, const float* x, float* y, void* hidden, float* hist_new, float* out, int T, float eps, hipStream_t s) {
  float* hn = B.hist ? hist_new : nullptr;
  constexpr int NT = in_threads<C>();
  constexpr size_t lds = InLay<C, TRV, NT>::LDS;
  hipLaunchKernelGGL((ffn_in_kernel<C, TRV, false, NT>), dim3(4 * C / 32, (T + TRV - 1) / TRV), dim3(NT), lds, s, x, y, hidden, hn, T, B, eps);
  hipLaunchKernelGGL((ffn_out_kernel<C, NW>), dim3(C / 16, (T + TR2 - 1) / TR2), dim3(64 * NW), 0, s, reinterpret_cast<const bf16_t*>(hidden), y, out, hn, T, B);
  return hipGetLastError() == hipSuccess ? 1 : vv_set_error(VV_E_HIP, "vv_convffn: launch failed");
}

int g_trv512 = 8, g_trv256 = 16, g_trv128 = 32;
int g_c128 = 1;

}

#ifdef VV_CF_TIMING
extern "C" int vv_convffn_debug_times(unsigned long long* out8, int reset) {
  if (hipMemcpyFromSymbol(out8, HIP_SYMBOL(g_cf_t), 8 * sizeof(unsigned long long)) != hipSuccess) return -1;
  if (reset) { unsigned long long z[8] = {0}; if (hipMemcpyToSymbol(HIP_SYMBOL(g_cf_t), z, sizeof(z)) != hipSuccess) return -1; }
  return 0;
}
#endif
void vv_convffn_set(int on) { g_on = on; }
void vv_convffn_set_rows(int c, int rows) { if (c == 512) g_trv512 = rows; else if (c == 256) g_trv256 = rows; else if (c == 128) g_trv128 = rows; }
void vv_convffn_set_c128(int on) { g_c128 = on; }
bool vv_convffn_prefers(int wdt, int T, int C) { return g_on && g_c128 && wdt == VV_BF16 && C == 128 && T >= 3 && T <= 1024; }
void vv_skinny_set(int on, int min_m, int max_m) { g_skinny = on; if (min_m > 0) g_skinny_min_m = min_m; if (max_m > 0) g_skinny_max_m = max_m; }

vv_skinny_route vv_skinny_decide(const vv_lin_args& a) {
  vv_skinny_route r = {0, 0, 0};
  if (!g_skinny || a.wdt != VV_BF16 || a.w2 || a.pro != VV_PRO_NONE || a.act != VV_ACT_NONE || a.gate || a.res || a.mod_scale || a.flags) return r;
  if (a.m < g_skinny_min_m || a.m > g_skinny_max_m || a.n % 16 || a.ldx % 4 || a.ldx == 0 || ((uintptr_t)a.x % 16) || ((uintptr_t)a.w % 16)) return r;
  static const int table[7][3] = {{128, 1, 1}, {256, 2, 1}, {512, 4, 1}, {1024, 8, 1}, {2048, 16, 1}, {2560, 20, 1}, {5120, 20, 2}};
  for (const auto& t : table)
    if (a.k == t[0]) { r.kind = 1; r.nst = t[1]; r.nb = t[2]; }
  return r;
}

bool vv_skinny_covers(const vv_lin_args& a) { return vv_skinny_decide(a).kind != 0; }

int vv_skinny_route_name(const vv_skinny_route& r, char* name, int cap) { return snprintf(name, (size_t)cap, "skinny<nst=%d,nb=%d>", r.nst, r.nb); }

int vv_launch_skinny(const vv_lin_args& a, hipStream_t s) {
  const vv_skinny_route r = vv_skinny_decide(a);
  if (!r.kind) return 0;
  dim3 grid(a.n / 16, (a.m + 15) / 16);
  const bf16_t* W = reinterpret_cast<const bf16_t*>(a.w);
#define VV_SK(NSTV, NBV)                                                                                                                    \
  if (r.nst == NSTV && r.nb == NBV) {                                                                                                       \
    hipLaunchKernelGGL((skinny_kernel<NSTV, NBV>), grid, dim3(256), 0, s, a.x, a.ldx, a.m, W, a.k, a.bias, a.out, a.ldo);                   \
    return 1;                                                                                                                               \
  }
  VV_SK(1, 1) VV_SK(2, 1) VV_SK(4, 1) VV_SK(8, 1) VV_SK(16, 1) VV_SK(20, 1) VV_SK(20, 2)
#undef VV_SK
  return 0;
}

int vv_convffn_init() {
#define VV_CF_ATTR(CC, TT)                                                                                                                  \
  { constexpr int nt_ = in_threads<CC>(); constexpr int l_ = (int)InLay<CC, TT, nt_>::LDS;                                                 \
    if (hipFuncSetAttribute(reinterpret_cast<const void*>(&ffn_in_kernel<CC, TT, false, nt_>), hipFuncAttributeMaxDynamicSharedMemorySize, l_) != hipSuccess) \
      return vv_set_error(VV_E_HIP, "vv_convffn_init: cannot raise the LDS limit"); }
  VV_CF_ATTR(128, 16) VV_CF_ATTR(128, 32) VV_CF_ATTR(256, 8) VV_CF_ATTR(256, 16) VV_CF_ATTR(256, 32) VV_CF_ATTR(512, 8) VV_CF_ATTR(512, 16) VV_CF_ATTR(512, 32) VV_CF_ATTR(1024, 8)
#undef VV_CF_ATTR
  {
    constexpr int l1 = (int)InLay<2048, 1, 256>::LDS;
    if (hipFuncSetAttribute(reinterpret_cast<const void*>(&ffn_in_kernel<2048, 1, true, 256>), hipFuncAttributeMaxDynamicSharedMemorySize, l1) != hipSuccess)
      return vv_set_error(VV_E_HIP, "vv_convffn_init: cannot raise the LDS limit");
  }
  return 0;
}

int g_t1 = 1;
void vv_convffn_set_t1(int on) { g_t1 = on; }

int vv_launch_ffn_in_row(const vv_block& B, int wdt, const float* x, float* y, float* hidden, float* hist_new, int C, float eps, hipStream_t s) {
  if (!g_on || !g_t1 || wdt != VV_BF16 || C != 2048 || !B.hist) return 0;
  auto a16 = [](const void* q) { return q && ((uintptr_t)q % 16) == 0; };
  if (!a16(B.w1) || !a16(B.b1) || !a16(B.gamma) || !a16(B.norm_w) || !a16(B.ffn_norm_w) || !a16(B.dw_b) || !a16(B.dw_w) || !a16(x) || !a16(y) ||
      !a16(hidden) || !a16(hist_new) || !a16(B.hist) || x == y)
    return 0;
  constexpr size_t lds = InLay<2048, 1, 256>::LDS;
  hipLaunchKernelGGL((ffn_in_kernel<2048, 1, true, 256>), dim3(4 * 2048 / 32, 1), dim3(256), lds, s, x, y, hidden, hist_new, 1, B, eps);
  return hipGetLastError() == hipSuccess ? 1 : vv_set_error(VV_E_HIP, "vv_convffn: launch failed");
}

int g_t1hs = 1;
void vv_convffn_set_t1hs(int on) { g_t1hs = on; }

int vv_launch_ffn_in_row_hs(const vv_block& B, int wdt, const float* x, float* y, float* hidden, float* hist_new, int C, float eps, hipStream_t s) {
  if (!g_on || !g_t1 || !g_t1hs || wdt != VV_BF16 || C != 2048 || !B.hist || !B.hs || !B.dw_last) return 0;
  auto a16 = [](const void* q) { return q && ((uintptr_t)q % 16) == 0; };
  if (!a16(B.w1) || !a16(B.b1) || !a16(B.gamma) || !a16(B.norm_w) || !a16(B.ffn_norm_w) || !a16(B.dw_b) || !a16(B.dw_last) || !a16(B.hs) || !a16(x) ||
      !a16(y) || !a16(hidden) || !a16(hist_new) || !a16(B.hist) || x == y)
    return 0;
  if (!vv_launch_conv_hot_row(B, x, y, hidden, hist_new, C, eps, s))
    hipLaunchKernelGGL(ffn_in_row_kernel, dim3(4 * 2048 / 32), dim3(256), 0, s, x, y, hidden, hist_new, B, eps);
  return hipGetLastError() == hipSuccess ? 1 : vv_set_error(VV_E_HIP, "vv_convffn: launch failed");
}

static int convffn_decide(const vv_block& B, int wdt, const float* x, const float* y, const void* hidden, const float* hist_new, const float* out, int T,
                          int C, int* trv, int* nw) {
  if (!g_on || wdt != VV_BF16 || T < 3 || (C != 128 && C != 256 && C != 512 && C != 1024) || (C == 1024 && T > 64)) return 0;
  if (C == 128 ? (!g_c128 || T > 1024) : T > 256) return 0;
  auto a16 = [](const void* q) { return q && ((uintptr_t)q % 16) == 0; };
  if (!a16(B.w1) || !a16(B.w2) || !a16(B.b1) || !B.b2 || !a16(B.gamma) || !B.ffn_gamma || !a16(B.norm_w) || !a16(B.ffn_norm_w) || !a16(B.dw_b) ||
      !a16(B.dw_w) || !a16(x) || !a16(y) || !a16(hidden) || !a16(hist_new) || !out || (B.hist && !a16(B.hist)))
    return 0;
  {
    const uintptr_t xa = (uintptr_t)x, ya = (uintptr_t)y, bytes = (uintptr_t)T * C * 4;
    if (xa < ya + bytes && ya < xa + bytes) return 0;
  }
  *nw = 4;
  if (C == 128) *trv = g_trv128 == 16 ? 16 : 32;
  else if (C == 256) *trv = (g_trv256 == 8 || g_trv256 == 16) ? g_trv256 : 32;
  else if (C == 512) *trv = (g_trv512 == 8 || g_trv512 == 16) ? g_trv512 : 32;
  else { *trv = 8; *nw = 8; }
  return 1;
}

int vv_launch_convffn(const vv_block& B, int wdt, const float* x, float* y, void* hidden, float* hist_new, float* out, int T, int C, float eps,
                      hipStream_t s) {
  int trv = 0, nw = 0;
  if (!convffn_decide(B, wdt, x, y, hidden, hist_new, out, T, C, &trv, &nw)) return 0;
#define VV_CF_GO(CC, TT, NN) if (C == CC && trv == TT) return launch_c<CC, TT, NN>(B, x, y, hidden, hist_new, out, T, eps, s)
  VV_CF_GO(128, 16, 4); VV_CF_GO(128, 32, 4);
  VV_CF_GO(256, 8, 4); VV_CF_GO(256, 16, 4); VV_CF_GO(256, 32, 4);
  VV_CF_GO(512, 8, 4); VV_CF_GO(512, 16, 4); VV_CF_GO(512, 32, 4);
  VV_CF_GO(1024, 8, 8);
#undef VV_CF_GO
  return vv_set_error(VV_E_UNSUPPORTED, "vv_convffn: no kernel for C=%d with %d-row tiles", C, trv);
}

static int block_mid_decide(const vv_block* b, int wdt, const float* x, const float* out, void* ws, int T, int C, float** y, char** hidden, float** hn,
                            int* trv, int* nw) {
  if (!b || !x || !out || !ws || T <= 0) return vv_set_error(VV_E_ARG, "vv_block_mid: bad args");
  *y = reinterpret_cast<float*>(ws);
  *hidden = reinterpret_cast<char*>(ws) + (size_t)T * C * 4;
  *hn = reinterpret_cast<float*>(*hidden + (size_t)T * 4 * C * 2);
  if (!convffn_decide(*b, wdt, x, *y, *hidden, *hn, out, T, C, trv, nw))
    return vv_set_error(VV_E_UNSUPPORTED, "vv_block_mid: shape not covered (C=%d T=%d wdt=%d)", C, T, wdt);
  return 0;
}

extern "C" size_t vv_block_mid_ws_bytes(int T, int C) { return (size_t)T * C * 4 + (size_t)T * 4 * C * 2 + (size_t)HALO * C * 4 + 64; }

extern "C" int vv_block_mid(const vv_block* b, int wdt, const float* x, float* out, void* ws, int T, int C, float eps, vv_stream_t stream) {
  float* y; char* hidden; float* hn;
  int trv = 0, nw = 0;
  VV_TRY(block_mid_decide(b, wdt, x, out, ws, T, C, &y, &hidden, &hn, &trv, &nw));
  const int rc = vv_launch_convffn(*b, wdt, x, y, hidden, hn, out, T, C, eps, (hipStream_t)stream);
  return rc < 0 ? rc : 0;
}

extern "C" int vv_block_mid_route(const vv_block* b, int wdt, const float* x, const float* out, const void* ws, int T, int C, char* name, int cap) {
  if (!name || cap <= 0) return vv_set_error(VV_E_ARG, "vv_block_mid_route: no room for the name");
  name[0] = 0;
  float* y; char* hidden; float* hn;
  int trv = 0, nw = 0;
  VV_TRY(block_mid_decide(b, wdt, x, out, const_cast<void*>(ws), T, C, &y, &hidden, &hn, &trv, &nw));
  snprintf(name, (size_t)cap, "ffn_in<c=%d,trv=%d,nt=%d> + ffn_out<c=%d,nw=%d>", C, trv, in_threads_of(C), C, nw);
  return 0;
}
```

### vibevoice_rocm_amd/csrc/vv_kernels.hip

```cpp
#include <hip/hip_runtime.h>
#include <hip/hip_bf16.h>
#include <stdint.h>
#include <stdio.h>
#include <string.h>
#include <math.h>

#include "vv_hip.h"
#include "vv_common.h"
#include "vv_device.h"

static thread_local char g_err[512] = "";

int vv_set_error(int code, const char* fmt, ...) {
  va_list ap;
  va_start(ap, fmt);
  vsnprintf(g_err, sizeof(g_err), fmt, ap);
  va_end(ap);
  return code;
}

extern "C" const char* vv_last_error(void) { return g_err; }
extern "C" int vv_abi_version(void) { return 6; }
int vv_mixer_init();
extern "C" int vv_init(void) {
  VV_TRY(vv_mixer_init());
  VV_TRY(vv_mfma_gemm_init());
  VV_TRY(vv_gemm_packed_init());
  VV_TRY(vv_block1d_init());
  VV_TRY(vv_convffn_init());
  VV_TRY(vv_gemv_rows_init());
  return vv_fused_init();
}
static float* g_rows_part = nullptr;
static int* g_rows_tk = nullptr;
static const size_t G_ROWS_PART_FLOATS = (size_t)4 << 20, G_ROWS_TICKETS = 4096;
static int rows_scratch(int on) {
  if (on && !g_rows_part) {
    if (hipMalloc(&g_rows_part, G_ROWS_PART_FLOATS * sizeof(float)) != hipSuccess || hipMalloc(&g_rows_tk, G_ROWS_TICKETS * sizeof(int)) != hipSuccess ||
        hipMemset(g_rows_tk, 0, G_ROWS_TICKETS * sizeof(int)) != hipSuccess)
      return vv_set_error(VV_E_HIP, "vv_tune: gemv_rows_scratch allocation failed");
  }
  if (!on && g_rows_part) { (void)hipFree(g_rows_part); (void)hipFree(g_rows_tk); g_rows_part = nullptr; g_rows_tk = nullptr; }
  return 0;
}
void vv_gemv_rows_set_dbg(int d);
void vv_gemv_rows_set_atomic(int on);
void vv_gemv_stream_set_blocks(int b);
void vv_gemv_stream_set_waves(int w);
void vv_gemv_stream_set_opt(int o);
void vv_gemv_stream_set_long(int cap, int ku);
void vv_gemv_stream_set_dual_rw(int r);
void vv_gemv_stream_set_small_rw(int r);
void vv_mfma_set_mt(int mt);
void vv_mfma_set_tiled_rows(int r);
void vv_mfma_set_tiled_bk128(int on);
void vv_mfma_set_tiled_small(int t);
void vv_mfma_set_tiled_dual_bk64(int on);
void vv_mfma_set_tiled_small_dual(int t);
void vv_mfma_set_tiled_small_k(int k);
void vv_mixer_set_rows(int on);
void vv_mfma_set_mt_prefill(int mt);
extern int g_attn_group;
void vv_attn_decode_set_gqa(int on);
void vv_attn_decode_set_gqa_keys(int k);
extern "C" int vv_tune(const char* key, int value) {
  if (key && !strcmp(key, "gemv_long_cap")) { vv_gemv_stream_set_long(value, 0); return 0; }
  if (key && !strcmp(key, "gemv_long_ku")) { vv_gemv_stream_set_long(0, value); return 0; }
  if (key && !strcmp(key, "gemv_blocks")) { vv_gemv_stream_set_blocks(value); vv_gemv_mx6_set_blocks(value); return 0; }
  if (key && !strcmp(key, "gemv_waves")) { vv_gemv_stream_set_waves(value); return 0; }
  if (key && !strcmp(key, "gemv_rows")) { vv_gemv_rows_set(value, 0, -1); return 0; }
  if (key && !strcmp(key, "gemv_rows_blocks")) { vv_gemv_rows_set(-1, value, -1); return 0; }
  if (key && !strcmp(key, "gemv_rows_pers")) { vv_gemv_rows_set(-1, 0, value); return 0; }
  if (key && !strcmp(key, "gemv_rows_scratch")) return rows_scratch(value);
  if (key && !strcmp(key, "gemv_rows_dbg")) { vv_gemv_rows_set_dbg(value); return 0; }
  if (key && !strcmp(key, "gemv_rows_atomic")) { vv_gemv_rows_set_atomic(value); return 0; }
  if (key && !strcmp(key, "gemv_opt")) { vv_gemv_stream_set_opt(value); return 0; }
  if (key && !strcmp(key, "gemv_dual_rw")) { vv_gemv_stream_set_dual_rw(value); return 0; }
  if (key && !strcmp(key, "gemv_small_rw")) { vv_gemv_stream_set_small_rw(value); return 0; }
  if (key && !strcmp(key, "gemv_hot")) { vv_gemv_hot_set(value); return 0; }
  if (key && !strcmp(key, "conv_hot")) { vv_conv_hot_set(value); return 0; }
  if (key && !strcmp(key, "mixer_rows")) { vv_mixer_set_rows(value); return 0; }
  if (key && !strcmp(key, "block1d_fused")) { vv_block1d_set_fused(value); return 0; }
  if (key && !strcmp(key, "block1d_blocks")) { vv_block1d_set_blocks(value); return 0; }
  if (key && !strcmp(key, "convffn")) { vv_convffn_set(value); return 0; }
  if (key && !strcmp(key, "convffn_t1")) { vv_convffn_set_t1(value); return 0; }
  if (key && !strcmp(key, "convffn_t1hs")) { vv_convffn_set_t1hs(value); return 0; }
  if (key && !strcmp(key, "convffn_rows512")) { vv_convffn_set_rows(512, value); return 0; }
  if (key && !strcmp(key, "convffn_rows256")) { vv_convffn_set_rows(256, value); return 0; }
  if (key && !strcmp(key, "convffn_rows128")) { vv_convffn_set_rows(128, value); return 0; }
  if (key && !strcmp(key, "convffn_c128")) { vv_convffn_set_c128(value); return 0; }
  if (key && !strcmp(key, "skinny")) { vv_skinny_set(value, 0, 0); return 0; }
  if (key && !strcmp(key, "skinny_min_m")) { vv_skinny_set(1, value, 0); return 0; }
  if (key && !strcmp(key, "skinny_max_m")) { vv_skinny_set(1, 0, value); return 0; }
  if (key && !strcmp(key, "mfma_tiled_bk128")) { vv_mfma_set_tiled_bk128(value); return 0; }
  if (key && !strcmp(key, "attn_group")) { g_attn_group = value; return 0; }
  if (key && !strcmp(key, "attn_gqa")) { vv_attn_decode_set_gqa(value); return 0; }
  if (key && !strcmp(key, "attn_gqa_keys")) { vv_attn_decode_set_gqa_keys(value); return 0; }
  if (key && !strcmp(key, "mfma_tiled_small_k")) { vv_mfma_set_tiled_small_k(value); return 0; }
  if (key && !strcmp(key, "mfma_tiled_dual_bk64")) { vv_mfma_set_tiled_dual_bk64(value); return 0; }
  if (key && !strcmp(key, "mfma_tiled_small_dual")) { vv_mfma_set_tiled_small_dual(value); return 0; }
  if (key && !strcmp(key, "mfma_tiled_small")) { vv_mfma_set_tiled_small(value); return 0; }
  if (key && !strcmp(key, "mfma_tiled_rows")) { vv_mfma_set_tiled_rows(value); return 0; }
  if (key && !strcmp(key, "gemm_packed_rows")) { vv_gemm_packed_set_rows(value); return 0; }
  if (key && !strcmp(key, "mfma_mt")) { vv_mfma_set_mt(value); return 0; }
  if (key && !strcmp(key, "mfma_mt_prefill")) { vv_mfma_set_mt_prefill(value); return 0; }
  return vv_set_error(VV_E_ARG, "vv_tune: unknown key");
}

__device__ __forceinline__ float bf2f(unsigned int u16) { return __uint_as_float(u16 << 16); }
__device__ __forceinline__ float wave_sum(float v) {
#pragma unroll
  for (int o = 32; o > 0; o >>= 1) v += __shfl_xor(v, o);
  return v;
}

template <typename WT> struct WL;
template <> struct WL<float> {
  static __device__ __forceinline__ void load8(const float* p, float (&o)[8]) {
    const float4 a = *reinterpret_cast<const float4*>(p);
    const float4 b = *reinterpret_cast<const float4*>(p + 4);
    o[0] = a.x; o[1] = a.y; o[2] = a.z; o[3] = a.w; o[4] = b.x; o[5] = b.y; o[6] = b.z; o[7] = b.w;
  }
  static __device__ __forceinline__ void load4(const float* p, float (&o)[4]) {
    const float4 a = *reinterpret_cast<const float4*>(p);
    o[0] = a.x; o[1] = a.y; o[2] = a.z; o[3] = a.w;
  }
  static __device__ __forceinline__ float load1(const float* p) { return *p; }
};
template <> struct WL<bf16_t> {
  static __device__ __forceinline__ void load8(const bf16_t* p, float (&o)[8]) {
    const uint4 v = *reinterpret_cast<const uint4*>(p);
    unpack8(u32x4{v.x, v.y, v.z, v.w}, o);
  }
  static __device__ __forceinline__ void load4(const bf16_t* p, float (&o)[4]) {
    const uint2 v = *reinterpret_cast<const uint2*>(p);
    o[0] = __uint_as_float(v.x << 16); o[1] = __uint_as_float(v.x & 0xffff0000u);
    o[2] = __uint_as_float(v.y << 16); o[3] = __uint_as_float(v.y & 0xffff0000u);
  }
  static __device__ __forceinline__ float load1(const bf16_t* p) { return bf2f(*p); }
};

__device__ __forceinline__ void lin_epilogue(const vv_lin_args& a, int m, int n, float v, float v2) {
  a.out[(int64_t)m * a.ldo + n] = vv_epi_value(a, v, v2, EpiAtUse{a, m, n});
}

#define GEMV_THREADS 256

template <int M>
__device__ __forceinline__ void row_stats(const vv_lin_args& a, float* red, float (&rstd)[M]) {
  const int tid = threadIdx.x, lane = tid & 63, wave = tid >> 6;
  float ss[M];
#pragma unroll
  for (int m = 0; m < M; ++m) {
    const float* xr = a.x + (int64_t)m * a.ldx;
    float s = 0.f;
    for (int k = tid; k < a.k; k += GEMV_THREADS) { const float v = xr[k]; s += v * v; }
    ss[m] = wave_sum(s);
  }
  if (lane == 0) {
#pragma unroll
    for (int m = 0; m < M; ++m) red[wave * M + m] = ss[m];
  }
  __syncthreads();
#pragma unroll
  for (int m = 0; m < M; ++m) {
    const float t = red[m] + red[M + m] + red[2 * M + m] + red[3 * M + m];
    rstd[m] = rsqrtf(t / (float)a.k + a.eps);
  }
  __syncthreads();
}

template <int M>
__device__ __forceinline__ void stage_chunk(const vv_lin_args& a, float* xs, int kc0, int kc, int kcp, const float (&rstd)[M]) {
  for (int idx = threadIdx.x; idx < M * kcp; idx += GEMV_THREADS) {
    const int m = idx / kcp, kk = idx - m * kcp;
    float v = 0.f;
    if (kk < kc) {
      const int k = kc0 + kk;
      v = a.x[(int64_t)m * a.ldx + k];
      if (a.pro == VV_PRO_RMSNORM) {
        v *= rstd[m];
        if (a.norm_w) v *= a.norm_w[k];
        if (a.mod_scale) v = v * (1.0f + a.mod_scale[(int64_t)m * a.ld_mod + k]) + a.mod_shift[(int64_t)m * a.ld_mod + k];
      } else if (a.pro == VV_PRO_SILU) {
        v = vv_silu(v);
      }
    }
    xs[idx] = v;
  }
}

template <typename WT, int M, bool DUAL, int KSPLIT, int RW>
__global__ __launch_bounds__(GEMV_THREADS) void gemv_kernel(const vv_lin_args a, const int KC) {
  extern __shared__ __attribute__((aligned(16))) float smem[];
  float* red = smem;
  float* xs = smem + 64 * 4;
  const int tid = threadIdx.x, lane = tid & 63, wave = tid >> 6;
  const int K = a.k, N = a.n;
  const WT* __restrict__ W = reinterpret_cast<const WT*>(a.w);
  const WT* __restrict__ W2 = reinterpret_cast<const WT*>(a.w2);

  float rstd[M];
#pragma unroll
  for (int m = 0; m < M; ++m) rstd[m] = 1.f;
  if (a.pro == VV_PRO_RMSNORM) row_stats<M>(a, red, rstd);

  const int row0 = (KSPLIT == 1 ? (blockIdx.x * 4 + wave) : blockIdx.x) * RW;
  float acc[RW][M], acc2[DUAL ? RW : 1][M];
#pragma unroll
  for (int r = 0; r < RW; ++r)
#pragma unroll
    for (int m = 0; m < M; ++m) { acc[r][m] = 0.f; if (DUAL) acc2[r][m] = 0.f; }

  for (int kc0 = 0; kc0 < K; kc0 += KC) {
    const int kc = min(KC, K - kc0);
    const int kcp = (kc + 7) & ~7;
    if (kc0 > 0) __syncthreads();
    stage_chunk<M>(a, xs, kc0, kc, kcp, rstd);
    __syncthreads();
    const int kstart = (KSPLIT == 1 ? lane : (wave * 64 + lane)) * 8;
    const int kstep = (KSPLIT == 1 ? 64 : 256) * 8;
#pragma unroll 2
    for (int k = kstart; k < kc; k += kstep) {
      float w[RW][8], w2[DUAL ? RW : 1][8];
#pragma unroll
      for (int r = 0; r < RW; ++r) {
        const int n = min(row0 + r, N - 1);
        WL<WT>::load8(W + (int64_t)n * K + kc0 + k, w[r]);
        if (DUAL) WL<WT>::load8(W2 + (int64_t)n * K + kc0 + k, w2[r]);
      }
#pragma unroll
      for (int m = 0; m < M; ++m) {
        const float4 x0 = *reinterpret_cast<const float4*>(xs + m * kcp + k);
// ... 1801 lines not shown
```

### vibevoice_rocm_amd/csrc/vv_model.hip

```cpp
#include <hip/hip_runtime.h>
#include <stdint.h>
#include <string.h>

#include "vv_hip.h"
#include "vv_common.h"

namespace {

struct Carver {
  char* p;
  explicit Carver(void* base) : p(reinterpret_cast<char*>(base)) {}
  float* take(size_t n_floats) {
    float* r = reinterpret_cast<float*>(p);
    p += (n_floats * sizeof(float) + 255) & ~(size_t)255;
    return r;
  }
};
inline size_t al(size_t n_floats) { return (n_floats * sizeof(float) + 255) & ~(size_t)255; }

inline vv_lin_args lin_base(const float* x, int64_t ldx, int m, const void* w, int n, int k, int wdt, float* out, int64_t ldo) {
  vv_lin_args a;
  memset(&a, 0, sizeof(a));
  a.x = x; a.ldx = ldx; a.m = m; a.w = w; a.n = n; a.k = k; a.wdt = wdt; a.out = out; a.ldo = ldo;
  return a;
// ... 476 lines not shown
    if (pre < 0) return pre;
  }
  vv_lin_args a;
  if (!pre) {
    a = lin_base(cond2, ld_cond, 2, h->cond_proj, D, h->cond_dim, h->wdt, c0, D);
    VV_TRY(vv_linear(&a, stream));
    if (cb) VV_TRY(vv_add_rows_silu_bf16(c0, D, temb, D, c, 2 * n_steps, 2, D, stream));
    else VV_TRY(vv_add_rows_silu(c0, D, temb, D, c, 2 * n_steps, 2, D, stream));
  }
  VV_TRY(head_modulations(h, c, 2 * n_steps, mod, modf, true, cb, stream));
  if (rt.step_ku) {
    float* hb[2] = {hcur, hcur2};
    if (!pre) VV_TRY(vv_head_init_fused(h, noise, Xs, Ms, hb[0], D, s));
    for (int i = 0; i < n_steps; ++i) {
      float* hc = hb[i & 1];
      for (int l = 0; l < h->layers; ++l) {
        const vv_head_layer& L = h->layer[l];
        const float* ml = mod[l] + (size_t)2 * i * 3 * D;
        a = lin_base(hc, D, 2, L.wgate, h->ffn, D, h->wdt, act, h->ffn);
        a.pro = VV_PRO_RMSNORM; a.norm_w = L.norm_w; a.eps = h->eps;
        a.mod_shift = ml; a.mod_scale = ml + D; a.ld_mod = 3 * D;
        a.w2 = L.wup; a.act = VV_ACT_SWIGLU; a.flags = VV_LIN_W_REUSED;
        use_w8(a, wq, L.q_gate, &L.q_up);
        VV_TRY(vv_linear(&a, stream));
        a = lin_base(act, h->ffn, 2, L.wdown, D, h->ffn, h->wdt, hc, D);
        a.gate = ml + 2 * D; a.gate_ld = 3 * D; a.res = hc; a.ldres = D; a.flags = VV_LIN_W_REUSED;
        use_w8(a, wq, L.q_down);
        VV_TRY(vv_linear(&a, stream));
      }
      const float* mf = modf + (size_t)2 * i * 2 * D;
      VV_TRY(vv_head_boundary_fused(h, hc, D, mf, mf + D, 2 * D, cfg_scale, &coef[i], Xs, Ms, hb[(i + 1) & 1], D, latent_out, s));
    }
    return 0;
  }
  for (int i = 0; i <= n_steps; ++i) {
    const float* xin = (i == 0) ? noise : xb[(i - 1) & 1];
    float* xout = (i == n_steps) ? latent_out : xb[i & 1];
    VV_TRY(vv_dpm_proj(i == 0 ? nullptr : v, h->latent, cfg_scale, i == 0 ? nullptr : &coef[i - 1], xin, mb[(i - 1) & 1], xout, mb[i & 1],
                       i == n_steps ? nullptr : h->noisy_proj, h->wdt, h->latent, D, hcur, D, 2,
                       (sde_noise && i > 0) ? sde_noise + (size_t)(i - 1) * h->latent : nullptr, stream));
    if (i == n_steps) break;
    VV_TRY(head_body(h, wq, nullptr, 0, 2, mod, modf, 2 * (int64_t)i, hcur, act, v, stream));
  }
  (void)s;
  return 0;
}

extern "C" size_t vv_head_ws_bytes_batch(const vv_head* h, int n_steps, int B) {
  if (!h || n_steps <= 0 || B <= 0 || B > 8) return 0;
  if (h->layers < 0 || h->layers > 16) return 0;
  VV_WQ_STRIP(vv_head, h);
  return head_carve_batch(h, n_steps, B, false).end;
}

extern "C" size_t vv_head_ws_bytes_batch_sde(const vv_head* h, int n_steps, int B) {
  if (!vv_head_ws_bytes_batch(h, n_steps, B)) return 0;
  VV_WQ_STRIP(vv_head, h);
  return head_carve_batch(h, n_steps, B, true).end;
}

static int head_sample_batch(const char* sde_fn, const vv_head* h, const float* cond, int64_t ld_cond, const float* noise, int64_t ld_noise, const float* temb,
                             const vv_dpm_coef* coef, int n_steps, float cfg_scale, float* latent_out, int64_t ld_latent, int B, void* ws,
                             const float* sde_noise, int64_t ld_sde, vv_stream_t stream, const float* cfg_rows = nullptr) {
  const char* fn = sde_fn ? sde_fn : "vv_head_sample_batch";
  if (!noise || !latent_out) return vv_set_error(VV_E_ARG, "%s: null pointer", fn);
  HeadRoute rt;
  VV_TRY(head_batch_decide(fn, sde_fn != nullptr, h, cond, temb, coef, n_steps, B, sde_noise != nullptr, ld_sde, cfg_rows != nullptr, ws, &rt));
  VV_WQ_STRIP(vv_head, h);
  const bool f8q = wq == VV_FP8;
  hipStream_t s = (hipStream_t)stream;
  const int D = h->D, R2 = 2 * B;
  const size_t R = (size_t)R2 * n_steps;
  const HeadWs o = head_carve_batch(h, n_steps, B, sde_noise != nullptr);
  auto at = [&](size_t off) { return reinterpret_cast<float*>(reinterpret_cast<char*>(ws) + off); };
  float* c0 = at(o.c0);
  float* c = at(o.c);
  float* mod[16];
  for (int l = 0; l < h->layers; ++l) mod[l] = at(o.mod[l]);
  float* modf = at(o.modf);
  float* hb[2] = {at(o.hb[0]), at(o.hb[1])};
  float* act = at(o.act);
  const int64_t sst = D + h->latent;
  float* Xs = at(o.Xs);
  float* Ms = at(o.Ms);
  const size_t rpart_n = o.rpart_n, rtick_n = o.rtick_n;
  float* rpart = at(o.rpart);
  int* rtick = reinterpret_cast<int*>(at(o.rtick));
  if (hipMemsetAsync(rtick, 0, rtick_n * sizeof(int), s) != hipSuccess) return vv_set_error(VV_E_HIP, "%s: memset", fn);
  float* NX = sde_noise ? at(o.NX) : nullptr;
  if (NX) VV_TRY(vv_head_sde_proj_fused(h, sde_noise, ld_sde, n_steps, B, NX, s));
  vv_lin_args a = lin_base(cond, ld_cond, R2, h->cond_proj, D, h->cond_dim, h->wdt, c0, D);
  VV_TRY(vv_linear_ws(&a, nullptr, nullptr, rpart, rpart_n, rtick, rtick_n, stream, nullptr, nullptr, fragq));
  VV_TRY(vv_add_rows_silu_bf16(c0, D, temb, D, c, (int)R, R2, D, stream));
  VV_TRY(head_modulations(h, c, (int)R, mod, modf, true, true, stream));
  for (int b = 0; b < B; ++b)
    VV_TRY(vv_head_init_fused(h, noise + (size_t)b * ld_noise, Xs + (size_t)b * sst, Ms + (size_t)b * sst, hb[0] + (size_t)2 * b * D, D, s));
  for (int i = 0; i < n_steps; ++i) {
    float* hc = hb[i & 1];
    for (int l = 0; l < h->layers; ++l) {
      const vv_head_layer& L = h->layer[l];
      const float* ml = mod[l] + (size_t)R2 * i * 3 * D;
      a = lin_base(hc, D, R2, L.wgate, h->ffn, D, h->wdt, act, h->ffn);
      a.pro = VV_PRO_RMSNORM; a.norm_w = L.norm_w; a.eps = h->eps;
      a.mod_shift = ml; a.mod_scale = ml + D; a.ld_mod = 3 * D;
      a.w2 = L.wup; a.act = VV_ACT_SWIGLU; a.flags = VV_LIN_W_REUSED;
      VV_TRY(vv_linear_ws(&a, L.f_gate, L.f_up, rpart, rpart_n, rtick, rtick_n, stream, f8q ? &L.q_gate : nullptr, f8q ? &L.q_up : nullptr, fragq));
      a = lin_base(act, h->ffn, R2, L.wdown, D, h->ffn, h->wdt, hc, D);
      a.gate = ml + 2 * D; a.gate_ld = 3 * D; a.res = hc; a.ldres = D; a.flags = VV_LIN_W_REUSED;
      VV_TRY(vv_linear_ws(&a, L.f_down, nullptr, rpart, rpart_n, rtick, rtick_n, stream, f8q ? &L.q_down : nullptr, nullptr, fragq));
    }
    const float* mf = modf + (size_t)R2 * i * 2 * D;
    VV_TRY(vv_head_boundary_batch(h, hc, D, mf, mf + D, 2 * D, cfg_scale, &coef[i], Xs, Ms, sst, hb[(i + 1) & 1], D, latent_out, ld_latent, B, s,
                                  NX ? NX + (size_t)i * sst : nullptr, (int64_t)n_steps * sst, cfg_rows));
  }
  return 0;
}

extern "C" int vv_head_sample_batch(const vv_head* h, const float* cond, int64_t ld_cond, const float* noise, int64_t ld_noise, const float* temb,
                                    const vv_dpm_coef* coef, int n_steps, float cfg_scale, float* latent_out, int64_t ld_latent, int B, void* ws,
                                    vv_stream_t stream) {
  return head_sample_batch(nullptr, h, cond, ld_cond, noise, ld_noise, temb, coef, n_steps, cfg_scale, latent_out, ld_latent, B, ws,
                           nullptr, 0, stream);
}

extern "C" int vv_head_sample_batch_sde(const vv_head* h, const float* cond, int64_t ld_cond, const float* noise, int64_t ld_noise, const float* temb,
                                        const vv_dpm_coef* coef, int n_steps, float cfg_scale, float* latent_out, int64_t ld_latent, int B, void* ws,
                                        const float* sde_noise, int64_t ld_sde, vv_stream_t stream) {
  return head_sample_batch("vv_head_sample_batch_sde", h, cond, ld_cond, noise, ld_noise, temb, coef, n_steps, cfg_scale, latent_out, ld_latent, B, ws,
                           sde_noise, ld_sde, stream);
}

extern "C" int vv_head_sample_batch_cfg(const vv_head* h, const float* cond, int64_t ld_cond, const float* noise, int64_t ld_noise, const float* temb,
                                        const vv_dpm_coef* coef, int n_steps, const float* cfg_rows, float* latent_out, int64_t ld_latent, int B, void* ws,
                                        const float* sde_noise, int64_t ld_sde, vv_stream_t stream) {
  if (!cfg_rows) return vv_set_error(VV_E_ARG, "vv_head_sample_batch_cfg: null cfg_rows");
  return head_sample_batch("vv_head_sample_batch_cfg", h, cond, ld_cond, noise, ld_noise, temb, coef, n_steps, 0.f, latent_out, ld_latent, B, ws,
                           sde_noise, ld_sde, stream, cfg_rows);
}

static inline int conv_ctx_of(const vv_conv& c) { return c.transposed ? 1 : c.kk - c.stride; }

static void convnet_sizes(const vv_convnet* net, int64_t t_in, int decoder, size_t* act_elems, size_t* hid_elems) {
  size_t amax = 0, hmax = 0;
  int64_t T = t_in;
  for (int i = 0; i < net->n_stages; ++i) {
    const vv_conv& cv = net->sample[i];
    const int ctx = conv_ctx_of(cv);
    size_t in_el = (size_t)(T + ctx + cv.kk + cv.stride) * cv.cin;
    if (in_el > amax) amax = in_el;
    if (cv.transposed) T = T * cv.stride; else T = (T + cv.stride - 1) / cv.stride;
    const size_t C = cv.cout;
    size_t el = (size_t)(T + 8) * C;
    if (el > amax) amax = el;
    if (net->n_blocks[i] > 0 && (size_t)T * 4 * C > hmax) hmax = (size_t)T * 4 * C;
  }
  size_t in_el = (size_t)(T + 8 + net->head.kk) * net->head.cin;
  if (in_el > amax) amax = in_el;
  (void)decoder;
  *act_elems = amax + 64;
  *hid_elems = hmax + 64;
}

static bool convnet_streaming(const vv_convnet* net) {
  for (int i = 0; i <= net->n_stages; ++i) {
    const vv_conv& cv = (i == net->n_stages) ? net->head : net->sample[i];
    if (conv_ctx_of(cv) > 0 && !cv.state) return false;
  }
  return true;
}
static size_t convnet_pad_floats(const vv_convnet* net, int64_t t_in, size_t* offs ) {
  size_t tot = 0;
  int64_t T = t_in;
  for (int i = 0; i <= net->n_stages; ++i) {
    const vv_conv& cv = (i == net->n_stages) ? net->head : net->sample[i];
    if (offs) offs[i] = tot;
    tot += (((size_t)(T + conv_ctx_of(cv) + 2) * cv.cin) + 63) & ~(size_t)63;
    if (cv.transposed) T = T * cv.stride; else T = (T + cv.stride - 1) / cv.stride;
  }
  return tot;
}

#define VV_ROW_BLOCKS 16
#define VV_ROW_HIST_FLOATS ((size_t)VV_ROW_BLOCKS * 6 * 2048)
#define VV_CTX_ITEMS (VV_MAX_STAGES + 1 + 16)

extern "C" size_t vv_convnet_ws_bytes(const vv_convnet* net, int64_t t_in, int decoder) {
  if (!net || t_in <= 0) return 0;
  VV_WQ_STRIP(vv_convnet, net);
  size_t a, h;
  convnet_sizes(net, t_in, decoder, &a, &h);
  return 2 * al(a) + al(h) + (convnet_streaming(net) ? al(convnet_pad_floats(net, t_in, nullptr)) + al(VV_ROW_HIST_FLOATS) : 0);
}

static int run_blocks(const vv_convnet* net, int wq, int stage, int64_t T, int C, float*& cur, float*& other, float* hid,
                      int nctx, float** pad_out, vv_stream_t stream, float* next_pad = nullptr, float* row_hist = nullptr,
                      vv_conv_ctx_item* items = nullptr, int* n_items = nullptr, int* row_stage = nullptr) {
  const int nb = net->n_blocks[stage];
  for (int j = 0; j < nb; ++j) {
    const vv_block& B = net->blocks[stage][j];
    const bool last = (j == nb - 1);
    if (!vv_convffn_prefers(net->wdt, (int)T, C)) {
      float* dst = last ? (next_pad ? next_pad : other) + (size_t)nctx * C : other;
      const int fused = vv_launch_block1d(B, net->wdt, cur, dst, (int)T, C, net->eps, (hipStream_t)stream);
      if (fused < 0) return fused;
      if (fused) {
        if (last) { *pad_out = next_pad ? next_pad : other; cur = nullptr; }
        else { float* t = cur; cur = other; other = t; }
        continue;
      }
    }
    float* final_dst = last ? (next_pad ? next_pad : cur) + (size_t)nctx * C : nullptr;
    if (last) *pad_out = next_pad ? next_pad : cur;
    if (T == 1 && row_hist && items && n_items && j < VV_ROW_BLOCKS && B.hist && !B.q_w1.q && *n_items < VV_CTX_ITEMS &&
        (*row_stage < 0 || *row_stage == stage)) {
      float* hn = row_hist + (size_t)j * 6 * C;
      int one = vv_launch_ffn_in_row_hs(B, net->wdt, cur, other, hid, hn, C, net->eps, (hipStream_t)stream);
      if (one == 0) one = vv_launch_ffn_in_row(B, net->wdt, cur, other, hid, hn, C, net->eps, (hipStream_t)stream);
      if (one < 0) return one;
      if (one) {
        *row_stage = stage;
        items[(*n_items)++] = vv_conv_ctx_item{hn, B.hist, 6, 0, C, B.dw_w, B.hs};
        float* dst1 = (last && final_dst) ? final_dst : other;
        vv_lin_args a1 = lin_base(hid, 4 * C, 1, B.w2, C, 4 * C, net->wdt, dst1, C);
        a1.bias = B.b2; a1.gate = B.ffn_gamma; a1.gate_ld = 0; a1.res = other; a1.ldres = C;
        use_w8(a1, wq, B.q_w2);
        VV_TRY(vv_linear(&a1, stream));
        if (dst1 == other) { float* t = cur; cur = other; other = t; }
        else { cur = nullptr; }
        continue;
      }
    }
    if (B.hs && B.hist && items && n_items) {
      if (*n_items >= VV_CTX_ITEMS) return vv_set_error(VV_E_UNSUPPORTED, "convnet: more than %d streaming-state moves in one net", VV_CTX_ITEMS);
      items[(*n_items)++] = vv_conv_ctx_item{B.hist, B.hist, 6, 0, C, B.dw_w, B.hs};
    }
    {
      float* dst2 = (last && final_dst) ? final_dst : other;
      const int two = vv_launch_convffn(B, net->wdt, cur, other, hid, reinterpret_cast<float*>(reinterpret_cast<char*>(hid) + (size_t)T * 4 * C * 2),
                                        dst2, (int)T, C, net->eps, (hipStream_t)stream);
      if (two < 0) return two;
      if (two) {
        if (dst2 == other) { float* t = cur; cur = other; other = t; }
        else { cur = nullptr; }
        continue;
      }
    }
    VV_TRY(vv_block_mixer(cur, other, (int)T, C, B.norm_w, net->eps, B.dw_w, B.dw_b, B.gamma, B.hist, stream));
    const bool handoff = net->wdt == VV_BF16 && T > 8 && C % 16 == 0 && ((uintptr_t)B.w1 % 16 == 0) && ((uintptr_t)B.w2 % 16 == 0);
    vv_lin_args a;
    const long tiles1 = (long)((4 * C) / 128) * ((T + 127) / 128);
    if (handoff && C % 32 == 0 && (4 * C) % 128 == 0 && T >= 64 && tiles1 >= 24) {
      void* xb = reinterpret_cast<char*>(hid) + (size_t)T * 4 * C * 2;
      VV_TRY(vv_cast_rows_bf16(other, C, (int)T, C, VV_PRO_RMSNORM, B.ffn_norm_w, net->eps, xb, C, stream));
      a = lin_base((const float*)xb, C, (int)T, B.w1, 4 * C, C, net->wdt, hid, 4 * C);
      a.flags = VV_LIN_X_BF16; a.bias = B.b1; a.act = VV_ACT_GELU;
    } else {
      a = lin_base(other, C, (int)T, B.w1, 4 * C, C, net->wdt, hid, 4 * C);
      a.pro = VV_PRO_RMSNORM; a.norm_w = B.ffn_norm_w; a.eps = net->eps; a.bias = B.b1; a.act = VV_ACT_GELU;
    }
    if (handoff) a.flags |= VV_LIN_OUT_BF16;
    use_w8(a, wq, B.q_w1);
    VV_TRY(vv_linear(&a, stream));
    float* dst = (j == nb - 1 && final_dst) ? final_dst : other;
    a = lin_base(hid, 4 * C, (int)T, B.w2, C, 4 * C, net->wdt, dst, C);
    if (handoff) a.flags |= VV_LIN_X_BF16;
    a.bias = B.b2; a.gate = B.ffn_gamma; a.gate_ld = 0; a.res = other; a.ldres = C;
    use_w8(a, wq, B.q_w2);
    VV_TRY(vv_linear(&a, stream));
    if (dst == other) { float* t = cur; cur = other; other = t; }
    else { cur = nullptr; }
  }
  return 0;
}

static int conv_left_ctx(const vv_conv& cv, float* pad, int64_t T, vv_stream_t stream) {
  const int ctx = conv_ctx_of(cv);
  if (ctx <= 0) return 0;
  if (cv.state) return vv_conv_ctx(pad, cv.state, ctx, (int)T, cv.cin, stream);
  hipError_t e = hipMemsetAsync(pad, 0, (size_t)ctx * cv.cin * 4, (hipStream_t)stream);
  if (e != hipSuccess) return vv_set_error(VV_E_HIP, "conv_left_ctx: %s", hipGetErrorString(e));
  return 0;
}

static int decoder_run(const char* who, const vv_convnet* net, const float* latent, int T0, float pre_scale, float pre_bias, float* wav,
                       void* ws, vv_stream_t stream, const float* mid) {
  if (!net || (!latent && !mid) || !wav || !ws) return vv_set_error(VV_E_ARG, "%s: null pointer", who);
  if (T0 <= 0 || net->n_stages < 1 || net->n_stages > VV_MAX_STAGES) return vv_set_error(VV_E_ARG, "%s: bad T/stages", who);
  VV_WQ_STRIP(vv_convnet, net);
  const int first = mid ? 1 : 0;
  size_t ael, hel;
  convnet_sizes(net, T0, 1, &ael, &hel);
  Carver cvr(ws);
  float* A = cvr.take(ael);
  float* Bf = cvr.take(ael);
  float* hid = cvr.take(hel);
  int64_t T = T0;
  const vv_conv& stem = net->sample[0];
  if (stem.transposed || stem.stride != 1) return vv_set_error(VV_E_ARG, "%s: stem must be a stride-1 conv", who);
  const bool streaming = convnet_streaming(net);
  if (mid && (!streaming || net->n_stages < 2 || !net->sample[1].transposed))
    return vv_set_error(VV_E_UNSUPPORTED, "%s: needs a streaming net whose second conv is the transposed hand-over", who);
  size_t poff[VV_MAX_STAGES + 1];
  float* pads = nullptr;
  vv_conv_ctx_item items[VV_CTX_ITEMS];
  int n_items = 0, row_stage = -1;
  float* row_hist = nullptr;
  if (streaming) {
    pads = cvr.take(convnet_pad_floats(net, T0, poff));
    row_hist = cvr.take(VV_ROW_HIST_FLOATS);
    int64_t Ti = T0;
    for (int i = 0; i <= net->n_stages; ++i) {
      const vv_conv& cv = (i == net->n_stages) ? net->head : net->sample[i];
      if (conv_ctx_of(cv) > 0 && (!mid || i > 1)) items[n_items++] = vv_conv_ctx_item{pads + poff[i], cv.state, conv_ctx_of(cv), (int)Ti, cv.cin};
      if (cv.transposed) Ti *= cv.stride;
    }
    vv_conv_ctx_item gi[VV_MAX_STAGES + 2];
    for (int i = 0; i < n_items; ++i) gi[i] = items[i];
    int n_gather = n_items;
    if (!mid)
      gi[n_gather++] = vv_conv_ctx_item{pads + poff[0] + (size_t)conv_ctx_of(stem) * stem.cin, const_cast<float*>(latent), (int)T, 0, stem.cin, nullptr, nullptr, 1,
                                        pre_scale, pre_bias};
    VV_TRY(vv_conv_ctx_batch(gi, n_gather, 0, (hipStream_t)stream));
  }
  float* pad = streaming ? pads + poff[0] : A;
  if (!streaming) VV_TRY(vv_affine(latent, pre_scale, pre_bias, pad + (size_t)conv_ctx_of(stem) * stem.cin, (int64_t)T * stem.cin, stream));
  float* cur = nullptr;
  float* other = nullptr;
  for (int i = first; i < net->n_stages; ++i) {
    const vv_conv& cv = net->sample[i];
    if (!streaming) VV_TRY(conv_left_ctx(cv, pad, T, stream));
    float* outb = (pad == A) ? Bf : A;
    vv_lin_args a;
    if (mid && i == 1) {
      outb = A;
      T *= cv.stride;
      hipError_t e = hipMemcpyAsync(outb, mid, (size_t)T * cv.cout * 4, hipMemcpyDeviceToDevice, (hipStream_t)stream);
      if (e != hipSuccess) return vv_set_error(VV_E_HIP, "%s: %s", who, hipGetErrorString(e));
    } else if (cv.transposed) {
      a = lin_base(pad, cv.cin, (int)T, cv.w, cv.stride * cv.cout, 2 * cv.cin, net->wdt, outb, (int64_t)cv.stride * cv.cout);
      a.bias = cv.b;
      VV_TRY(vv_linear(&a, stream));
      T *= cv.stride;
    } else {
      a = lin_base(pad, (int64_t)cv.stride * cv.cin, (int)T, cv.w, cv.cout, cv.kk * cv.cin, net->wdt, outb, cv.cout);
      a.bias = cv.b;
      VV_TRY(vv_linear(&a, stream));
    }
    cur = outb;
    other = (cur == A) ? Bf : A;
    const int C = cv.cout;
    const vv_conv& nxt = (i + 1 < net->n_stages) ? net->sample[i + 1] : net->head;
    const int nctx = conv_ctx_of(nxt);
    float* next_pad = streaming ? pads + poff[i + 1] : nullptr;
    if (net->n_blocks[i] > 0) {
      VV_TRY(run_blocks(net, wq, i, T, C, cur, other, hid, nctx, &pad, stream, next_pad, row_hist, items, &n_items, &row_stage));
    } else {
      float* dstb = next_pad ? next_pad : other;
      hipError_t e = hipMemcpyAsync(dstb + (size_t)nctx * C, cur, (size_t)T * C * 4, hipMemcpyDeviceToDevice, (hipStream_t)stream);
      if (e != hipSuccess) return vv_set_error(VV_E_HIP, "%s: %s", who, hipGetErrorString(e));
      pad = dstb;
    }
  }
  const vv_conv& hd = net->head;
  if (!streaming) VV_TRY(conv_left_ctx(hd, pad, T, stream));
  vv_lin_args a = lin_base(pad, (int64_t)hd.stride * hd.cin, (int)T, hd.w, hd.cout, hd.kk * hd.cin, net->wdt, wav, hd.cout);
  a.bias = hd.b;
  VV_TRY(vv_linear(&a, stream));
  if (streaming) VV_TRY(vv_conv_ctx_batch(items, n_items, 1, (hipStream_t)stream));
  return 0;
}

extern "C" int vv_decoder_forward(const vv_convnet* net, const float* latent, int T0, float pre_scale, float pre_bias, float* wav,
                                  void* ws, vv_stream_t stream) {
  if (!latent) return vv_set_error(VV_E_ARG, "vv_decoder_forward: null pointer");
  return decoder_run("vv_decoder_forward", net, latent, T0, pre_scale, pre_bias, wav, ws, stream, nullptr);
}

extern "C" int vv_decoder_forward_from(const vv_convnet* net, const float* mid, float* wav, void* ws, vv_stream_t stream) {
  if (!mid) return vv_set_error(VV_E_ARG, "vv_decoder_forward_from: null pointer");
  return decoder_run("vv_decoder_forward_from", net, nullptr, 1, 0.f, 0.f, wav, ws, stream, mid);
}

static int encoder_run(const char* who, const vv_convnet* net, const float* wav, int64_t T0, float* feat, void* ws, vv_stream_t stream, float* mid_out) {
  if (!net || !wav || (!feat && !mid_out) || !ws) return vv_set_error(VV_E_ARG, "%s: null pointer", who);
  if (T0 <= 0 || net->n_stages < 1 || net->n_stages > VV_MAX_STAGES) return vv_set_error(VV_E_ARG, "%s: bad T/stages", who);
  VV_WQ_STRIP(vv_convnet, net);
  const int last_i = mid_out ? net->n_stages - 2 : net->n_stages;
  hipStream_t s = (hipStream_t)stream;
  size_t ael, hel;
  convnet_sizes(net, T0, 0, &ael, &hel);
  Carver cvr(ws);
// ... 374 lines not shown
```

Baseline: 44.17 audio-sec/s.

## Add fused mid8 conv block path: f32 FFN-in kernel plus register GEMV with history copy

Adds a specialised path for convnet blocks with C=1024 and T=8 rows. It runs the existing ffn_in kernel with f32 hidden output, then a new GEMV kernel for w2 that holds weights and inputs in registers and applies bias, gate and residual in its epilogue. One extra block in the same grid copies the streaming history, so no separate copy is needed. The ffn_in kernel and layout are moved into a shared include file, and the workspace grows by 6*C floats to hold the new history buffer. This is meant to cut launch count and the MFMA-tile waste of the general convffn path for tiny T, at the cost of more code paths and an f32 hidden round-trip.

```diff
diff --git a/include/vv_hip.h b/include/vv_hip.h
--- a/include/vv_hip.h
+++ b/include/vv_hip.h
@@ -298,6 +298,11 @@
 typedef struct vv_conv_hot_shape { const char* name; int kind, m, n, k, bias, gate, res; } vv_conv_hot_shape;
 int vv_conv_hot_shapes(vv_conv_hot_shape* out, int cap);
 
+int vv_conv_mid8_shapes(vv_conv_hot_shape* out, int cap);
+int vv_conv_mid8_route(const struct vv_block* b, int wdt, const float* x, const float* out, const void* ws, int T, int C, char* name, int cap);
+size_t vv_conv_mid8_ws_bytes(int T);
+int vv_conv_mid8_block(const struct vv_block* b, int wdt, const float* x, float* out, void* ws, int T, int C, float eps, vv_stream_t stream);
+
 size_t vv_sizeof(const char* struct_name);
 
 #ifdef __cplusplus
diff --git a/vibevoice_rocm_amd/_lib.py b/vibevoice_rocm_amd/_lib.py
--- a/vibevoice_rocm_amd/_lib.py
+++ b/vibevoice_rocm_amd/_lib.py
@@ -193,6 +193,10 @@
     "vv_graph_destroy": (C.c_int, [vp]),
     "vv_nf4_import": (C.c_int, [C.POINTER(Nf4Src), vp, i64, C.c_int, C.c_int, vp, vp, vp]),
     "vv_conv_hot_shapes": (C.c_int, [vp, C.c_int]),
+    "vv_conv_mid8_shapes": (C.c_int, [vp, C.c_int]),
+    "vv_conv_mid8_route": (C.c_int, [vp, C.c_int, vp, vp, vp, C.c_int, C.c_int, C.c_char_p, C.c_int]),
+    "vv_conv_mid8_ws_bytes": (C.c_size_t, [C.c_int]),
+    "vv_conv_mid8_block": (C.c_int, [vp, C.c_int, vp, vp, vp, C.c_int, C.c_int, C.c_float, vp]),
     "vv_sizeof": (C.c_size_t, [C.c_char_p]),
     "vv_prof_begin": (C.c_int, [C.c_int]),
     "vv_prof_end": (C.c_int, [C.POINTER(ProfEntry), C.c_int, C.POINTER(C.c_int)]),
diff --git a/vibevoice_rocm_amd/build.py b/vibevoice_rocm_amd/build.py
--- a/vibevoice_rocm_amd/build.py
+++ b/vibevoice_rocm_amd/build.py
@@ -12,7 +12,7 @@
                                                "vv_fused.hip", "vv_attn_decode.hip", "vv_attn_prefill.hip", "vv_model.hip",
                                                "vv_nf4_import.hip", "vv_kv_copy.hip", "vv_noise.hip")]
 HDR = [os.path.join(ROOT, "include", "vv_hip.h"), os.path.join(HERE, "csrc", "vv_common.h"), os.path.join(HERE, "csrc", "vv_device.h"),
-       os.path.join(HERE, "csrc", "vv_head_boundary.inc"),
+       os.path.join(HERE, "csrc", "vv_head_boundary.inc"), os.path.join(HERE, "csrc", "vv_convffn_in.inc"),
        os.path.join(HERE, "csrc", "vv_gemv_rows.h"), os.path.join(HERE, "csrc", "vv_gemv_rows_body.inc"), os.path.join(HERE, "csrc", "vv_gemv_rows_tile.inc"),
        os.path.join(HERE, "csrc", "vv_llm_tail.inc"), os.path.join(HERE, "csrc", "vv_llm_tail_fast.inc")]
 OUT = os.path.join(HERE, "libvv_hip.so")
diff --git a/vibevoice_rocm_amd/csrc/vv_common.h b/vibevoice_rocm_amd/csrc/vv_common.h
--- a/vibevoice_rocm_amd/csrc/vv_common.h
+++ b/vibevoice_rocm_amd/csrc/vv_common.h
@@ -68,6 +68,11 @@
 int vv_launch_conv_hot_gemv(const vv_lin_args& a, int idx, hipStream_t s);
 int vv_launch_conv_hot_row(const vv_block& B, const float* x, float* y, float* hidden, float* hist_new, int C, float eps, hipStream_t s);
 void vv_conv_hot_set(int mask);
+int vv_launch_conv_mid8(const vv_block& B, int wdt, const float* x, float* y, float* hidden, float* hist_new, float* out, int rows, int rows_max, int C,
+                        float eps, hipStream_t s);
+int vv_conv_mid8_init();
+void vv_conv_mid8_set(int mask);
+bool vv_convffn_enabled();
 int vv_launch_gemv_rows(const vv_lin_args& a, float* part, size_t part_floats, int* tickets, size_t n_tickets, hipStream_t s);
 struct vv_rows_route { int kind, dual, nw, ks, pers, wf, ksplit, spw, atomic, n_groups, gx, rt; };
 vv_rows_route vv_gemv_rows_decide(const vv_lin_args& a, bool have_ws, size_t part_floats, size_t n_tickets);
diff --git a/vibevoice_rocm_amd/csrc/vv_conv_hot.hip b/vibevoice_rocm_amd/csrc/vv_conv_hot.hip
--- a/vibevoice_rocm_amd/csrc/vv_conv_hot.hip
+++ b/vibevoice_rocm_amd/csrc/vv_conv_hot.hip
@@ -330,6 +330,88 @@
     for (int r = 0; r < rows_out; ++r) out[((int64_t)b * rows_out + r) * ldo + i] = v;
   }
 }
+
+template <int BT, int N, int K, int NW, int R>
+__global__ __launch_bounds__(64 * NW) void mid_gemv_kernel(const float* __restrict__ x, int64_t ldx, int M, const bf16_t* __restrict__ W,
+                                                           const float* __restrict__ bias, const float* __restrict__ gate, const float* res, int64_t ldres,
+                                                           float* out, int64_t ldo, const float* __restrict__ mv_src, float* __restrict__ mv_dst, int mv_n4) {
+  constexpr int KU = K / (512 * NW);
+  static_assert(K % (512 * NW) == 0 && N % R == 0 && R * BT <= 64 * NW, "whole units, whole channel sets, one epilogue thread per output");
+  __shared__ float part[NW][R * BT];
+  const int tid = threadIdx.x, lane = tid & 63;
+  const int wave = __builtin_amdgcn_readfirstlane(tid >> 6);
+  if (blockIdx.x == N / R) {
+    for (int e = tid; e < mv_n4; e += 64 * NW) reinterpret_cast<float4*>(mv_dst)[e] = reinterpret_cast<const float4*>(mv_src)[e];
+    return;
+  }
+  const int n0 = (int)blockIdx.x * R;
+  int koff[KU];
+#pragma unroll
+  for (int u = 0; u < KU; ++u) koff[u] = (wave + NW * u) * 512 + lane * 8;
+  float4 xa[BT][KU], xb[BT][KU];
+#pragma unroll
+  for (int b = 0; b < BT; ++b) {
+    const float* xp = x + (int64_t)min(b, M - 1) * ldx;
+#pragma unroll
+    for (int u = 0; u < KU; ++u) {
+      xa[b][u] = *reinterpret_cast<const float4*>(xp + koff[u]);
+      xb[b][u] = *reinterpret_cast<const float4*>(xp + koff[u] + 4);
+    }
+  }
+  const int et = tid < R * BT ? tid : 0;
+  const int er_ = et / BT, eb_ = et - er_ * BT;
+  const float ebias = bias[n0 + er_];
+  const float eg = gate[n0 + er_];
+  const float er = res[(int64_t)min(eb_, M - 1) * ldres + n0 + er_];
+  u32x4 wq[R][KU];
+#pragma unroll
+  for (int r = 0; r < R; ++r)
+#pragma unroll
+    for (int u = 0; u < KU; ++u) wq[r][u] = ldw<true>(W + (int64_t)(n0 + r) * K + koff[u]);
+  __builtin_amdgcn_sched_barrier(0);
+#pragma unroll
+  for (int b = 0; b < BT; ++b)
+#pragma unroll
+    for (int u = 0; u < KU; ++u) { VV_FENCE4(xa[b][u]); VV_FENCE4(xb[b][u]); }
+
+#pragma unroll
+  for (int b = 0; b < BT; ++b) {
+    vf2 p[R];
+#pragma unroll
+    for (int r = 0; r < R; ++r) p[r] = vf2{0.f, 0.f};
+#pragma unroll
+    for (int u = 0; u < KU; ++u) {
+      const float xr[8] = {xa[b][u].x, xa[b][u].y, xa[b][u].z, xa[b][u].w, xb[b][u].x, xb[b][u].y, xb[b][u].z, xb[b][u].w};
+#pragma unroll
+      for (int r = 0; r < R; ++r) fma_unit(wq[r][u], xr, p[r]);
+    }
+#pragma unroll
+    for (int r = 0; r < R; ++r) {
+      const float a = vv_wave_sum(p[r].x + p[r].y);
+      if (lane == 0) part[wave][r * BT + b] = a;
+    }
+  }
+  __syncthreads();
+  if (tid < R * BT) {
+    float s = 0.f;
+#pragma unroll
+    for (int w4 = 0; w4 < NW; ++w4) s += part[w4][tid];
+    const float v = gate_res(s + ebias, eg, er);
+    if (eb_ < M) out[(int64_t)eb_ * ldo + n0 + er_] = v;
+  }
+}
+
+#include "vv_convffn_in.inc"
+
+constexpr int MID_C = 1024, MID_T = 8, MID_NT = 512;
+constexpr size_t MID_IN_LDS = InLay<MID_C, MID_T, MID_NT>::LDS;
+
+constexpr int N_MID8 = 1;
+const vv_conv_hot_shape g_mid8_table[N_MID8] = {
+    {"mid8.w2", VV_CONV_HOT_GEMV, MID_T, MID_C, 4 * MID_C, 1,   1,   1},
+};
+constexpr int MID8_DEFAULT = 0x1;
+int g_mid8 = MID8_DEFAULT;
 
 constexpr int N_HOT = 4;
 const vv_conv_hot_shape g_table[N_HOT] = {
@@ -456,3 +538,79 @@
   VV_CHECK_LAUNCH("rows_bcast");
   return 0;
 }
+
+void vv_conv_mid8_set(int mask) { g_mid8 = mask < 0 ? MID8_DEFAULT : mask; }
+
+extern "C" int vv_conv_mid8_shapes(vv_conv_hot_shape* out, int cap) {
+  for (int i = 0; i < N_MID8 && i < cap; ++i) out[i] = g_mid8_table[i];
+  return N_MID8;
+}
+
+int vv_conv_mid8_init() {
+  if (hipFuncSetAttribute(reinterpret_cast<const void*>(&ffn_in_kernel<MID_C, MID_T, true, MID_NT>), hipFuncAttributeMaxDynamicSharedMemorySize, (int)MID_IN_LDS) != hipSuccess)
+    return vv_set_error(VV_E_HIP, "vv_conv_mid8_init: cannot raise the LDS limit");
+  return 0;
+}
+
+int vv_conv_mid8_covers(const vv_block& B, int wdt, const float* x, const float* y, const void* hidden, const float* hist_new, const float* out,
+                        int rows, int rows_max, int C) {
+  if (!(g_mid8 & 1) || !vv_convffn_enabled() || wdt != VV_BF16 || B.q_w1.q || B.q_w2.q || C != MID_C || rows < 1 || rows > rows_max || !B.hist) return 0;
+  if (!a16(B.w1) || !a16(B.w2) || !a16(B.b1) || !B.b2 || !a16(B.gamma) || !B.ffn_gamma || !a16(B.norm_w) || !a16(B.ffn_norm_w) || !a16(B.dw_b) || !a16(B.dw_w) ||
+      !a16(x) || !a16(y) || !a16(hidden) || !a16(hist_new) || !out || !a16(B.hist))
+    return 0;
+  const uintptr_t xa = (uintptr_t)x, ya = (uintptr_t)y, bytes = (uintptr_t)rows * C * 4;
+  if (xa < ya + bytes && ya < xa + bytes) return 0;
+  return 1;
+}
+
+int vv_launch_conv_mid8(const vv_block& B, int wdt, const float* x, float* y, float* hidden, float* hist_new, float* out, int rows, int rows_max, int C,
+                        float eps, hipStream_t s) {
+  if (!vv_conv_mid8_covers(B, wdt, x, y, hidden, hist_new, out, rows, rows_max, C)) return 0;
+  hipLaunchKernelGGL((ffn_in_kernel<MID_C, MID_T, true, MID_NT>), dim3(4 * MID_C / 32, 1), dim3(MID_NT), MID_IN_LDS, s, x, y, hidden, hist_new, rows, B, eps);
+  const bf16_t* W = reinterpret_cast<const bf16_t*>(B.w2);
+  const float* b2 = B.b2; const float* fg = B.ffn_gamma; const float* res = y; const float* mv = hist_new;
+  const int64_t ldh = 4 * MID_C, ld = MID_C;
+  if (g_mid8 & 256)
+    hipLaunchKernelGGL((mid_gemv_kernel<MID_T, MID_C, 4 * MID_C, 4, 4>), dim3(MID_C / 4 + 1), dim3(256), 0, s, hidden, ldh, rows, W, b2, fg, res, ld, out, ld, mv, B.hist,
+                       6 * MID_C / 4);
+  else
+    hipLaunchKernelGGL((mid_gemv_kernel<MID_T, MID_C, 4 * MID_C, 8, 4>), dim3(MID_C / 4 + 1), dim3(512), 0, s, hidden, ldh, rows, W, b2, fg, res, ld, out, ld, mv, B.hist,
+                       6 * MID_C / 4);
+  return hipGetLastError() == hipSuccess ? 1 : vv_set_error(VV_E_HIP, "vv_conv_mid8: launch failed");
+}
+
+static int mid8_carve(const vv_block* b, const float* x, const float* out, void* ws, int T, int C, float** y, float** hidden, float** hn) {
+  if (!b || !x || !out || !ws || T <= 0) return vv_set_error(VV_E_ARG, "vv_conv_mid8_block: bad args");
+  *y = reinterpret_cast<float*>(ws);
+  *hidden = *y + (size_t)T * C;
+  *hn = *hidden + (size_t)T * 4 * C;
+  return 0;
+}
+
+extern "C" size_t vv_conv_mid8_ws_bytes(int T) { return T < 1 || T > MID_T ? 0 : ((size_t)T * MID_C + (size_t)T * 4 * MID_C + (size_t)6 * MID_C) * 4 + 64; }
+
+extern "C" int vv_conv_mid8_block(const vv_block* b, int wdt, const float* x, float* out, void* ws, int T, int C, float eps, vv_stream_t stream) {
+  float *y, *hidden, *hn;
+  VV_TRY(mid8_carve(b, x, out, ws, T, C, &y, &hidden, &hn));
+  (void)vv_wq_strip(&wdt);
+  const int saved = g_mid8;
+  g_mid8 |= 1;
+  const int rc = vv_launch_conv_mid8(*b, wdt, x, y, hidden, hn, out, T, MID_T, C, eps, (hipStream_t)stream);
+  g_mid8 = saved;
+  if (rc == 0) return vv_set_error(VV_E_UNSUPPORTED, "vv_conv_mid8_block: not the mid8.w2 entry (C=%d T=%d wdt=%d)", C, T, wdt);
+  return rc < 0 ? rc : 0;
+}
+
+extern "C" int vv_conv_mid8_route(const vv_block* b, int wdt, const float* x, const float* out, const void* ws, int T, int C, char* name, int cap) {
+  if (!name || cap <= 0) return vv_set_error(VV_E_ARG, "vv_conv_mid8_route: no room for the name");
+  name[0] = 0;
+  float *y, *hidden, *hn;
+  int plain = wdt;
+  (void)vv_wq_strip(&plain);
+  if (b && x && out && ws && T > 0 && !mid8_carve(b, x, out, const_cast<void*>(ws), T, C, &y, &hidden, &hn) &&
+      vv_conv_mid8_covers(*b, plain, x, y, hidden, hn, out, T, T == MID_T ? MID_T : 0, C)) {
+    snprintf(name, (size_t)cap, "ffn_in_f32<c=%d,trv=%d,nt=%d> + mid_gemv<bt=%d,n=%d,k=%d,nw=%d,r=4>", MID_C, MID_T, MID_NT, MID_T, MID_C, 4 * MID_C, (g_mid8 & 256) ? 4 : 8);
+    return 0;
+  }
+  return vv_block_mid_route(b, wdt, x, out, ws, T, C, name, cap);
+}
diff --git a/vibevoice_rocm_amd/csrc/vv_convffn.hip b/vibevoice_rocm_amd/csrc/vv_convffn.hip
--- a/vibevoice_rocm_amd/csrc/vv_convffn.hip
+++ b/vibevoice_rocm_amd/csrc/vv_convffn.hip
@@ -17,249 +17,10 @@
 #endif
 
 constexpr int TR2 = 16;
-constexpr int HALO = 6;
 
 __device__ __forceinline__ float sq4(const float4 v) { return v.x * v.x + v.y * v.y + v.z * v.z + v.w * v.w; }
 
-template <int C, int TRV, int NT = 256> struct InLay {
-  static constexpr int VW = C >= 256 ? 4 : 2;
-  static constexpr int F4 = C / 4;
-  static constexpr int FV = C / VW;
-  static constexpr int TPR = FV < NT ? FV : NT;
-  static constexpr int NWV = NT / 64;
-  static constexpr int CPT = FV / TPR;
-  static constexpr int RP = NT / TPR;
-  static constexpr int NI = (TRV + HALO + RP - 1) / RP;
-  static constexpr int WR = NI * RP;
-  static constexpr int WPR = TPR / 64;
-  static constexpr int P1 = C + 8;
-  static constexpr int ST = C / (16 * NWV);
-  static constexpr size_t XN = (size_t)WR * C * 4;
-  static constexpr size_t RED = (size_t)NWV * 16 * 64 * 4;
-  static constexpr size_t XH = (size_t)(WR - HALO) * P1 * 2;
-  static constexpr size_t PART = (size_t)2 * WR * 8 * 4;
-  static constexpr size_t LDS = (XN > RED ? XN : RED) + XH + PART;
-};
-
-template <int VW> __device__ __forceinline__ void ldv(const float* p, float (&o)[VW]) {
-  if constexpr (VW == 4) { const float4 t = *reinterpret_cast<const float4*>(p); o[0] = t.x; o[1] = t.y; o[2] = t.z; o[3] = t.w; }
-  else { const float2 t = *reinterpret_cast<const float2*>(p); o[0] = t.x; o[1] = t.y; }
-}
-template <int VW> __device__ __forceinline__ void stv(float* p, const float (&o)[VW]) {
-  if constexpr (VW == 4) *reinterpret_cast<float4*>(p) = make_float4(o[0], o[1], o[2], o[3]);
-  else *reinterpret_cast<float2*>(p) = make_float2(o[0], o[1]);
-}
-
-template <int C, int TRV, bool HF32, int NT>
-__global__ __launch_bounds__(NT) void ffn_in_kernel(const float* __restrict__ x, float* __restrict__ y, void* __restrict__ hidden_v,
-                                                     float* __restrict__ hist_new, int T, const vv_block B, float eps) {
-  using L = InLay<C, TRV, NT>;
-  constexpr int TR = TRV, CPT = L::CPT, VW = L::VW, NWV = L::NWV;
-#ifdef VV_CF_TIMING
-  long long tprev_ = wall_clock64();
-#endif
-  extern __shared__ __attribute__((aligned(16))) unsigned char smem[];
-  float* xn = reinterpret_cast<float*>(smem);
-  float* red = reinterpret_cast<float*>(smem);
-  bf16_t* xh = reinterpret_cast<bf16_t*>(smem + (L::XN > L::RED ? L::XN : L::RED));
-  float* part = reinterpret_cast<float*>(smem + (L::XN > L::RED ? L::XN : L::RED) + L::XH);
-  float* part2 = part + L::WR * 8;
-  const int tid = threadIdx.x, lane = tid & 63, wave = __builtin_amdgcn_readfirstlane(tid >> 6);
-  const int n0 = blockIdx.x * 32;
-  const int t0 = blockIdx.y * TR;
-  const int rows = min(TR, T - t0);
-  const int lm = lane & 31, hk = (lane >> 5) * 8;
-
-  const int rloc = wave / L::WPR, slot = wave % L::WPR;
-  int c0[CPT];
-#pragma unroll
-  for (int j = 0; j < CPT; ++j) c0[j] = VW * (tid % L::TPR + L::TPR * j);
-  const float* hb = B.hist ? B.hist : x;
-  const float hkeep = B.hist ? 1.f : 0.f;
-  float own[L::NI][CPT][VW];
-#pragma unroll
-  for (int i = 0; i < L::NI; ++i) {
-    const int w = rloc + L::RP * i, t = t0 - HALO + w;
-    const bool isx = t >= 0;
-    const float* src = isx ? x + (int64_t)min(t, T - 1) * C : hb + (int64_t)(B.hist ? HALO + t : 0) * C;
-    const float keep = (w < rows + HALO) ? (isx ? 1.f : hkeep) : 0.f;
-#pragma unroll
-    for (int j = 0; j < CPT; ++j) {
-      ldv<VW>(src + c0[j], own[i][j]);
-#pragma unroll
-      for (int e = 0; e < VW; ++e) own[i][j][e] *= keep;
-    }
-  }
-  float nw[CPT][VW], db[CPT][VW], gm[CPT][VW], fw[CPT][VW];
-  float tap[CPT][VW * 7];
-#pragma unroll
-  for (int j = 0; j < CPT; ++j) {
-    ldv<VW>(B.norm_w + c0[j], nw[j]);
-    ldv<VW>(B.dw_b + c0[j], db[j]);
-    ldv<VW>(B.gamma + c0[j], gm[j]);
-    ldv<VW>(B.ffn_norm_w + c0[j], fw[j]);
-#pragma unroll
-    for (int q = 0; q < 7; ++q) {
-      float tq[VW];
-      ldv<VW>(B.dw_w + (size_t)c0[j] * 7 + VW * q, tq);
-#pragma unroll
-      for (int e = 0; e < VW; ++e) tap[j][VW * q + e] = tq[e];
-    }
-  }
-  u32x4 wf[L::ST];
-  {
-    const bf16_t* wr = reinterpret_cast<const bf16_t*>(B.w1) + (int64_t)(n0 + lm) * C + wave * (C / NWV) + hk;
-#pragma unroll
-    for (int s = 0; s < L::ST; ++s) wf[s] = *reinterpret_cast<const u32x4*>(wr + s * 16);
-  }
-  const int eg = wave & 3;
-  const float4 b1v = *reinterpret_cast<const float4*>(B.b1 + n0 + 8 * eg + 4 * (lane >> 5));
-  __builtin_amdgcn_sched_barrier(0);
-
-  CSTAMP(0);
-#pragma unroll
-  for (int i = 0; i < L::NI; ++i) {
-    const int w = rloc + L::RP * i;
-    float q = 0.f;
-#pragma unroll
-    for (int j = 0; j < CPT; ++j)
-#pragma unroll
-      for (int e = 0; e < VW; ++e) q = fmaf(own[i][j][e], own[i][j][e], q);
-    const float s = vv_wave_sum(q);
-    if (lane == 0) part[w * 8 + slot] = s;
-  }
-  __syncthreads();
-  CSTAMP(1);
-#pragma unroll
-  for (int i = 0; i < L::NI; ++i) {
-    const int w = rloc + L::RP * i, t = t0 - HALO + w;
-    float ss = part[w * 8];
-#pragma unroll
-    for (int sl = 1; sl < L::WPR; ++sl) ss += part[w * 8 + sl];
-    const bool isx = t >= 0;
-    const float rstd = isx ? rsqrtf(ss / (float)C + eps) : 1.f;
-#pragma unroll
-    for (int j = 0; j < CPT; ++j) {
-      float o[VW];
-#pragma unroll
-      for (int e = 0; e < VW; ++e) o[e] = own[i][j][e] * rstd * (isx ? nw[j][e] : 1.f);
-      stv<VW>(xn + w * C + c0[j], o);
-    }
-  }
-  __syncthreads();
-  CSTAMP(2);
-
-  float y1[L::NI][CPT][VW];
-#pragma unroll
-  for (int i = 0; i < L::NI; ++i) {
-#pragma unroll
-    for (int j = 0; j < CPT; ++j)
-#pragma unroll
-      for (int e = 0; e < VW; ++e) y1[i][j][e] = 0.f;
-    if (L::RP * i + L::RP - 1 < HALO) continue;
-    const int w = rloc + L::RP * i, tt = w - HALO;
-    const int tc = max(tt, 0);
-    const float ok = (tt >= 0 && tt < rows) ? 1.f : 0.f;
-    float q = 0.f;
-#pragma unroll
-    for (int j = 0; j < CPT; ++j) {
-      float s[VW];
-#pragma unroll
-      for (int e = 0; e < VW; ++e) s[e] = db[j][e];
-#pragma unroll
-      for (int k = 0; k < 7; ++k) {
-        float v[VW];
-        ldv<VW>(xn + (tc + k) * C + c0[j], v);
-#pragma unroll
-        for (int e = 0; e < VW; ++e) s[e] = fmaf(tap[j][7 * e + k], v[e], s[e]);
-      }
-#pragma unroll
-      for (int e = 0; e < VW; ++e) {
-        y1[i][j][e] = (own[i][j][e] + gm[j][e] * s[e]) * ok;
-        q = fmaf(y1[i][j][e], y1[i][j][e], q);
-      }
-    }
-    const float s2 = vv_wave_sum(q);
-    if (lane == 0) part2[w * 8 + slot] = s2;
-  }
-  if (hist_new && blockIdx.x == 0 && t0 + TR >= T) {
-    for (int e = tid; e < HALO * L::F4; e += NT) {
-      const int j = e / L::F4, c4 = e - j * L::F4;
-      *reinterpret_cast<float4*>(hist_new + (size_t)j * C + 4 * c4) = *reinterpret_cast<const float4*>(xn + (size_t)(T - t0 + j) * C + 4 * c4);
-    }
-  }
-  __syncthreads();
-  CSTAMP(3);
-  {
-    const int ys0 = blockIdx.x * (C / (int)gridDim.x);
-#pragma unroll
-    for (int i = 0; i < L::NI; ++i) {
-      if (L::RP * i + L::RP - 1 < HALO) continue;
-      const int w = rloc + L::RP * i, tt = w - HALO;
-      if (tt >= 0) {
-        float ss = part2[w * 8];
-#pragma unroll
-        for (int sl = 1; sl < L::WPR; ++sl) ss += part2[w * 8 + sl];
-        const float rstd = rsqrtf(ss / (float)C + eps);
-#pragma unroll
-        for (int j = 0; j < CPT; ++j) {
-          if constexpr (VW == 4) {
-            uint2 p;
-            p.x = pack2(y1[i][j][0] * rstd * fw[j][0], y1[i][j][1] * rstd * fw[j][1]);
-            p.y = pack2(y1[i][j][2] * rstd * fw[j][2], y1[i][j][3] * rstd * fw[j][3]);
-            *reinterpret_cast<uint2*>(xh + tt * L::P1 + c0[j]) = p;
-          } else {
-            *reinterpret_cast<unsigned int*>(xh + tt * L::P1 + c0[j]) = pack2(y1[i][j][0] * rstd * fw[j][0], y1[i][j][1] * rstd * fw[j][1]);
-          }
-          const bool mine = c0[j] >= ys0 && c0[j] < ys0 + C / (int)gridDim.x;
-          if (mine && tt < rows) stv<VW>(y + (int64_t)(t0 + tt) * C + c0[j], y1[i][j]);
-        }
-      }
-    }
-  }
-  __syncthreads();
-
-  CSTAMP(4);
-  f32x16 acc;
-#pragma unroll
-  for (int i = 0; i < 16; ++i) acc[i] = 0.f;
-  {
-    const bf16_t* xf = xh + min(lm, TR - 1) * L::P1 + wave * (C / NWV) + hk;
-#pragma unroll
-    for (int s = 0; s < L::ST; ++s) {
-      const u32x4 xb = *reinterpret_cast<const u32x4*>(xf + s * 16);
-      acc = __builtin_amdgcn_mfma_f32_32x32x16_bf16(__builtin_bit_cast(bf16x8, wf[s]), __builtin_bit_cast(bf16x8, xb), acc, 0, 0, 0);
-    }
-  }
-#pragma unroll
-  for (int r = 0; r < 16; ++r) red[(wave * 16 + r) * 64 + lane] = acc[r];
-  __syncthreads();
-  CSTAMP(5);
-  {
-    const int m = lane & 31;
-    if (m < rows && wave < 4) {
-      float v[4];
-#pragma unroll
-      for (int i = 0; i < 4; ++i) {
-        float s = 0.f;
-#pragma unroll
-        for (int w4 = 0; w4 < NWV; ++w4) s += red[(w4 * 16 + 4 * eg + i) * 64 + lane];
-        v[i] = s;
-      }
-      const float g0 = vv_gelu_as(v[0] + b1v.x), g1 = vv_gelu_as(v[1] + b1v.y), g2 = vv_gelu_as(v[2] + b1v.z), g3 = vv_gelu_as(v[3] + b1v.w);
-      const int64_t ho = (int64_t)(t0 + m) * (4 * C) + n0 + 8 * eg + 4 * (lane >> 5);
-      if (HF32) {
-        *reinterpret_cast<float4*>(reinterpret_cast<float*>(hidden_v) + ho) = make_float4(g0, g1, g2, g3);
-      } else {
-        uint2 p;
-        p.x = pack2(g0, g1);
-        p.y = pack2(g2, g3);
-        *reinterpret_cast<uint2*>(reinterpret_cast<bf16_t*>(hidden_v) + ho) = p;
-      }
-    }
-  }
-  CSTAMP(6);
-}
+#include "vv_convffn_in.inc"
 
 
 __global__ __launch_bounds__(256) void ffn_in_row_kernel(const float* __restrict__ x, float* __restrict__ y, float* __restrict__ hidden,
@@ -500,6 +261,7 @@
 }
 #endif
 void vv_convffn_set(int on) { g_on = on; }
+bool vv_convffn_enabled() { return g_on != 0; }
 void vv_convffn_set_rows(int c, int rows) { if (c == 512) g_trv512 = rows; else if (c == 256) g_trv256 = rows; else if (c == 128) g_trv128 = rows; }
 void vv_convffn_set_c128(int on) { g_c128 = on; }
 bool vv_convffn_prefers(int wdt, int T, int C) { return g_on && g_c128 && wdt == VV_BF16 && C == 128 && T >= 3 && T <= 1024; }
diff --git a/vibevoice_rocm_amd/csrc/vv_convffn_in.inc b/vibevoice_rocm_amd/csrc/vv_convffn_in.inc
--- /dev/null
+++ b/vibevoice_rocm_amd/csrc/vv_convffn_in.inc
@@ -0,0 +1,245 @@
+#ifndef CSTAMP
+#define CSTAMP(i) do { } while (0)
+#endif
+
+constexpr int HALO = 6;
+
+template <int C, int TRV, int NT = 256> struct InLay {
+  static constexpr int VW = C >= 256 ? 4 : 2;
+  static constexpr int F4 = C / 4;
+  static constexpr int FV = C / VW;
+  static constexpr int TPR = FV < NT ? FV : NT;
+  static constexpr int NWV = NT / 64;
+  static constexpr int CPT = FV / TPR;
+  static constexpr int RP = NT / TPR;
+  static constexpr int NI = (TRV + HALO + RP - 1) / RP;
+  static constexpr int WR = NI * RP;
+  static constexpr int WPR = TPR / 64;
+  static constexpr int P1 = C + 8;
+  static constexpr int ST = C / (16 * NWV);
+  static constexpr size_t XN = (size_t)WR * C * 4;
+  static constexpr size_t RED = (size_t)NWV * 16 * 64 * 4;
+  static constexpr size_t XH = (size_t)(WR - HALO) * P1 * 2;
+  static constexpr size_t PART = (size_t)2 * WR * 8 * 4;
+  static constexpr size_t LDS = (XN > RED ? XN : RED) + XH + PART;
+};
+
+template <int VW> __device__ __forceinline__ void ldv(const float* p, float (&o)[VW]) {
+  if constexpr (VW == 4) { const float4 t = *reinterpret_cast<const float4*>(p); o[0] = t.x; o[1] = t.y; o[2] = t.z; o[3] = t.w; }
+  else { const float2 t = *reinterpret_cast<const float2*>(p); o[0] = t.x; o[1] = t.y; }
+}
+template <int VW> __device__ __forceinline__ void stv(float* p, const float (&o)[VW]) {
+  if constexpr (VW == 4) *reinterpret_cast<float4*>(p) = make_float4(o[0], o[1], o[2], o[3]);
+  else *reinterpret_cast<float2*>(p) = make_float2(o[0], o[1]);
+}
+
+template <int C, int TRV, bool HF32, int NT>
+__global__ __launch_bounds__(NT) void ffn_in_kernel(const float* __restrict__ x, float* __restrict__ y, void* __restrict__ hidden_v,
+                                                     float* __restrict__ hist_new, int T, const vv_block B, float eps) {
+  using L = InLay<C, TRV, NT>;
+  constexpr int TR = TRV, CPT = L::CPT, VW = L::VW, NWV = L::NWV;
+#ifdef VV_CF_TIMING
+  long long tprev_ = wall_clock64();
+#endif
+  extern __shared__ __attribute__((aligned(16))) unsigned char smem[];
+  float* xn = reinterpret_cast<float*>(smem);
+  float* red = reinterpret_cast<float*>(smem);
+  bf16_t* xh = reinterpret_cast<bf16_t*>(smem + (L::XN > L::RED ? L::XN : L::RED));
+  float* part = reinterpret_cast<float*>(smem + (L::XN > L::RED ? L::XN : L::RED) + L::XH);
+  float* part2 = part + L::WR * 8;
+  const int tid = threadIdx.x, lane = tid & 63, wave = __builtin_amdgcn_readfirstlane(tid >> 6);
+  const int n0 = blockIdx.x * 32;
+  const int t0 = blockIdx.y * TR;
+  const int rows = min(TR, T - t0);
+  const int lm = lane & 31, hk = (lane >> 5) * 8;
+
+  const int rloc = wave / L::WPR, slot = wave % L::WPR;
+  int c0[CPT];
+#pragma unroll
+  for (int j = 0; j < CPT; ++j) c0[j] = VW * (tid % L::TPR + L::TPR * j);
+  const float* hb = B.hist ? B.hist : x;
+  const float hkeep = B.hist ? 1.f : 0.f;
+  float own[L::NI][CPT][VW];
+#pragma unroll
+  for (int i = 0; i < L::NI; ++i) {
+    const int w = rloc + L::RP * i, t = t0 - HALO + w;
+    const bool isx = t >= 0;
+    const float* src = isx ? x + (int64_t)min(t, T - 1) * C : hb + (int64_t)(B.hist ? HALO + t : 0) * C;
+    const float keep = (w < rows + HALO) ? (isx ? 1.f : hkeep) : 0.f;
+#pragma unroll
+    for (int j = 0; j < CPT; ++j) {
+      ldv<VW>(src + c0[j], own[i][j]);
+#pragma unroll
+      for (int e = 0; e < VW; ++e) own[i][j][e] *= keep;
+    }
+  }
+  float nw[CPT][VW], db[CPT][VW], gm[CPT][VW], fw[CPT][VW];
+  float tap[CPT][VW * 7];
+#pragma unroll
+  for (int j = 0; j < CPT; ++j) {
+    ldv<VW>(B.norm_w + c0[j], nw[j]);
+    ldv<VW>(B.dw_b + c0[j], db[j]);
+    ldv<VW>(B.gamma + c0[j], gm[j]);
+    ldv<VW>(B.ffn_norm_w + c0[j], fw[j]);
+#pragma unroll
+    for (int q = 0; q < 7; ++q) {
+      float tq[VW];
+      ldv<VW>(B.dw_w + (size_t)c0[j] * 7 + VW * q, tq);
+#pragma unroll
+      for (int e = 0; e < VW; ++e) tap[j][VW * q + e] = tq[e];
+    }
+  }
+  u32x4 wf[L::ST];
+  {
+    const bf16_t* wr = reinterpret_cast<const bf16_t*>(B.w1) + (int64_t)(n0 + lm) * C + wave * (C / NWV) + hk;
+#pragma unroll
+    for (int s = 0; s < L::ST; ++s) wf[s] = *reinterpret_cast<const u32x4*>(wr + s * 16);
+  }
+  const int eg = wave & 3;
+  const float4 b1v = *reinterpret_cast<const float4*>(B.b1 + n0 + 8 * eg + 4 * (lane >> 5));
+  __builtin_amdgcn_sched_barrier(0);
+
+  CSTAMP(0);
+#pragma unroll
+  for (int i = 0; i < L::NI; ++i) {
+    const int w = rloc + L::RP * i;
+    float q = 0.f;
+#pragma unroll
+    for (int j = 0; j < CPT; ++j)
+#pragma unroll
+      for (int e = 0; e < VW; ++e) q = fmaf(own[i][j][e], own[i][j][e], q);
+    const float s = vv_wave_sum(q);
+    if (lane == 0) part[w * 8 + slot] = s;
+  }
+  __syncthreads();
+  CSTAMP(1);
+#pragma unroll
+  for (int i = 0; i < L::NI; ++i) {
+    const int w = rloc + L::RP * i, t = t0 - HALO + w;
+    float ss = part[w * 8];
+#pragma unroll
+    for (int sl = 1; sl < L::WPR; ++sl) ss += part[w * 8 + sl];
+    const bool isx = t >= 0;
+    const float rstd = isx ? rsqrtf(ss / (float)C + eps) : 1.f;
+#pragma unroll
+    for (int j = 0; j < CPT; ++j) {
+      float o[VW];
+#pragma unroll
+      for (int e = 0; e < VW; ++e) o[e] = own[i][j][e] * rstd * (isx ? nw[j][e] : 1.f);
+      stv<VW>(xn + w * C + c0[j], o);
+    }
+  }
+  __syncthreads();
+  CSTAMP(2);
+
+  float y1[L::NI][CPT][VW];
+#pragma unroll
+  for (int i = 0; i < L::NI; ++i) {
+#pragma unroll
+    for (int j = 0; j < CPT; ++j)
+#pragma unroll
+      for (int e = 0; e < VW; ++e) y1[i][j][e] = 0.f;
+    if (L::RP * i + L::RP - 1 < HALO) continue;
+    const int w = rloc + L::RP * i, tt = w - HALO;
+    const int tc = max(tt, 0);
+    const float ok = (tt >= 0 && tt < rows) ? 1.f : 0.f;
+    float q = 0.f;
+#pragma unroll
+    for (int j = 0; j < CPT; ++j) {
+      float s[VW];
+#pragma unroll
+      for (int e = 0; e < VW; ++e) s[e] = db[j][e];
+#pragma unroll
+      for (int k = 0; k < 7; ++k) {
+        float v[VW];
+        ldv<VW>(xn + (tc + k) * C + c0[j], v);
+#pragma unroll
+        for (int e = 0; e < VW; ++e) s[e] = fmaf(tap[j][7 * e + k], v[e], s[e]);
+      }
+#pragma unroll
+      for (int e = 0; e < VW; ++e) {
+        y1[i][j][e] = (own[i][j][e] + gm[j][e] * s[e]) * ok;
+        q = fmaf(y1[i][j][e], y1[i][j][e], q);
+      }
+    }
+    const float s2 = vv_wave_sum(q);
+    if (lane == 0) part2[w * 8 + slot] = s2;
+  }
+  if (hist_new && blockIdx.x == 0 && t0 + TR >= T) {
+    for (int e = tid; e < HALO * L::F4; e += NT) {
+      const int j = e / L::F4, c4 = e - j * L::F4;
+      *reinterpret_cast<float4*>(hist_new + (size_t)j * C + 4 * c4) = *reinterpret_cast<const float4*>(xn + (size_t)(T - t0 + j) * C + 4 * c4);
+    }
+  }
+  __syncthreads();
+  CSTAMP(3);
+  {
+    const int ys0 = blockIdx.x * (C / (int)gridDim.x);
+#pragma unroll
+    for (int i = 0; i < L::NI; ++i) {
+      if (L::RP * i + L::RP - 1 < HALO) continue;
+      const int w = rloc + L::RP * i, tt = w - HALO;
+      if (tt >= 0) {
+        float ss = part2[w * 8];
+#pragma unroll
+        for (int sl = 1; sl < L::WPR; ++sl) ss += part2[w * 8 + sl];
+        const float rstd = rsqrtf(ss / (float)C + eps);
+#pragma unroll
+        for (int j = 0; j < CPT; ++j) {
+          if constexpr (VW == 4) {
+            uint2 p;
+            p.x = pack2(y1[i][j][0] * rstd * fw[j][0], y1[i][j][1] * rstd * fw[j][1]);
+            p.y = pack2(y1[i][j][2] * rstd * fw[j][2], y1[i][j][3] * rstd * fw[j][3]);
+            *reinterpret_cast<uint2*>(xh + tt * L::P1 + c0[j]) = p;
+          } else {
+            *reinterpret_cast<unsigned int*>(xh + tt * L::P1 + c0[j]) = pack2(y1[i][j][0] * rstd * fw[j][0], y1[i][j][1] * rstd * fw[j][1]);
+          }
+          const bool mine = c0[j] >= ys0 && c0[j] < ys0 + C / (int)gridDim.x;
+          if (mine && tt < rows) stv<VW>(y + (int64_t)(t0 + tt) * C + c0[j], y1[i][j]);
+        }
+      }
+    }
+  }
+  __syncthreads();
+
+  CSTAMP(4);
+  f32x16 acc;
+#pragma unroll
+  for (int i = 0; i < 16; ++i) acc[i] = 0.f;
+  {
+    const bf16_t* xf = xh + min(lm, TR - 1) * L::P1 + wave * (C / NWV) + hk;
+#pragma unroll
+    for (int s = 0; s < L::ST; ++s) {
+      const u32x4 xb = *reinterpret_cast<const u32x4*>(xf + s * 16);
+      acc = __builtin_amdgcn_mfma_f32_32x32x16_bf16(__builtin_bit_cast(bf16x8, wf[s]), __builtin_bit_cast(bf16x8, xb), acc, 0, 0, 0);
+    }
+  }
+#pragma unroll
+  for (int r = 0; r < 16; ++r) red[(wave * 16 + r) * 64 + lane] = acc[r];
+  __syncthreads();
+  CSTAMP(5);
+  {
+    const int m = lane & 31;
+    if (m < rows && wave < 4) {
+      float v[4];
+#pragma unroll
+      for (int i = 0; i < 4; ++i) {
+        float s = 0.f;
+#pragma unroll
+        for (int w4 = 0; w4 < NWV; ++w4) s += red[(w4 * 16 + 4 * eg + i) * 64 + lane];
+        v[i] = s;
+      }
+      const float g0 = vv_gelu_as(v[0] + b1v.x), g1 = vv_gelu_as(v[1] + b1v.y), g2 = vv_gelu_as(v[2] + b1v.z), g3 = vv_gelu_as(v[3] + b1v.w);
+      const int64_t ho = (int64_t)(t0 + m) * (4 * C) + n0 + 8 * eg + 4 * (lane >> 5);
+      if (HF32) {
+        *reinterpret_cast<float4*>(reinterpret_cast<float*>(hidden_v) + ho) = make_float4(g0, g1, g2, g3);
+      } else {
+        uint2 p;
+        p.x = pack2(g0, g1);
+        p.y = pack2(g2, g3);
+        *reinterpret_cast<uint2*>(reinterpret_cast<bf16_t*>(hidden_v) + ho) = p;
+      }
+    }
+  }
+  CSTAMP(6);
+}
diff --git a/vibevoice_rocm_amd/csrc/vv_kernels.hip b/vibevoice_rocm_amd/csrc/vv_kernels.hip
--- a/vibevoice_rocm_amd/csrc/vv_kernels.hip
+++ b/vibevoice_rocm_amd/csrc/vv_kernels.hip
@@ -28,6 +28,7 @@
   VV_TRY(vv_gemm_packed_init());
   VV_TRY(vv_block1d_init());
   VV_TRY(vv_convffn_init());
+  VV_TRY(vv_conv_mid8_init());
   VV_TRY(vv_gemv_rows_init());
   return vv_fused_init();
 }
@@ -79,6 +80,7 @@
   if (key && !strcmp(key, "gemv_small_rw")) { vv_gemv_stream_set_small_rw(value); return 0; }
   if (key && !strcmp(key, "gemv_hot")) { vv_gemv_hot_set(value); return 0; }
   if (key && !strcmp(key, "conv_hot")) { vv_conv_hot_set(value); return 0; }
+  if (key && !strcmp(key, "conv_mid8")) { vv_conv_mid8_set(value); return 0; }
   if (key && !strcmp(key, "mixer_rows")) { vv_mixer_set_rows(value); return 0; }
   if (key && !strcmp(key, "block1d_fused")) { vv_block1d_set_fused(value); return 0; }
   if (key && !strcmp(key, "block1d_blocks")) { vv_block1d_set_blocks(value); return 0; }
diff --git a/vibevoice_rocm_amd/csrc/vv_model.hip b/vibevoice_rocm_amd/csrc/vv_model.hip
--- a/vibevoice_rocm_amd/csrc/vv_model.hip
+++ b/vibevoice_rocm_amd/csrc/vv_model.hip
@@ -652,7 +652,7 @@
     const size_t C = cv.cout;
     size_t el = (size_t)(T + 8) * C;
     if (el > amax) amax = el;
-    if (net->n_blocks[i] > 0 && (size_t)T * 4 * C > hmax) hmax = (size_t)T * 4 * C;
+    if (net->n_blocks[i] > 0 && (size_t)T * 4 * C + 6 * C > hmax) hmax = (size_t)T * 4 * C + 6 * C;
   }
   size_t in_el = (size_t)(T + 8 + net->head.kk) * net->head.cin;
   if (in_el > amax) amax = in_el;
@@ -736,7 +736,8 @@
     }
     {
       float* dst2 = (last && final_dst) ? final_dst : other;
-      const int two = vv_launch_convffn(B, net->wdt, cur, other, hid, reinterpret_cast<float*>(reinterpret_cast<char*>(hid) + (size_t)T * 4 * C * 2),
+      int two = T != 8 ? 0 : vv_launch_conv_mid8(B, net->wdt, cur, other, hid, hid + (size_t)T * 4 * C, dst2, 8, 8, C, net->eps, (hipStream_t)stream);
+      if (two == 0) two = vv_launch_convffn(B, net->wdt, cur, other, hid, reinterpret_cast<float*>(reinterpret_cast<char*>(hid) + (size_t)T * 4 * C * 2),
                                         dst2, (int)T, C, net->eps, (hipStream_t)stream);
       if (two < 0) return two;
       if (two) {
```

Measured after the change: 44.17 audio-sec/s. No clear change (-0.0%).
